# bd4sur/Nano

Measured on AMD Instinct MI355X. Metric: decode_tokens_per_sec, higher is better.
Workload: dtype i8

## Files before the change

### include/nano_mi355x.h

```cpp
#ifndef NANO_MI355X_H
#define NANO_MI355X_H

#include <stddef.h>
#include <stdint.h>

#ifdef __cplusplus
extern "C" {
#endif

#define NANO_ARCH_NANO  0u
#define NANO_ARCH_QWEN2 2u
#define NANO_ARCH_QWEN3 3u

#define NANO_QUANT_F32 0x00u
#define NANO_QUANT_Q80 0x80u
#define NANO_QUANT_Q4K 0x42u

#define NANO_HIP_OK        0
#define NANO_HIP_EINVAL   -1
#define NANO_HIP_ERUNTIME -2
#define NANO_HIP_ENODEV   -3
#define NANO_HIP_ENOMEM   -4

#define NANO_MAX_BATCH 64u
// ... 295 lines not shown
    const float *norm_w;
    const float *attn_part;
    const float *attn_ml;
    uint32_t attn_nsplit, attn_n_head, attn_hd;
    uint32_t use_gemm;
    uint32_t ordered;
    uint32_t *route_out;
    float *out;
    uint32_t out_slots;
    uint32_t out_stride;
    float *tile_max;
    uint32_t tile_slots;
    uint32_t tile_pairs;
    uint32_t *ntiles_out;
    uint32_t *argmax_out;
    const float *resid_add;
    uint32_t resid_add_stride;
} NanoFusedGemvDesc;
int nano_hip_op_fused_gemv(int device, const NanoFusedGemvDesc *d);

typedef struct NanoLoraOpDesc {
    uint32_t E, KD, rank, alpha, nb, S;
    uint32_t v_bstride, _pad;
    const float *x;
    const float *norm_w;
    const float *a[3], *b[3];
    const uint32_t *pos;
    float *q, *kraw, *v;
    uint64_t q_floats, k_floats, v_floats;
} NanoLoraOpDesc;
int nano_hip_op_lora_qkv(int device, const NanoLoraOpDesc *d);
int nano_hip_op_lora_o(int device, const NanoLoraOpDesc *d);
typedef struct NanoLoraAdapter {
    uint32_t rank, alpha;
    const float *a[3], *b[3];
} NanoLoraAdapter;
typedef struct NanoLoraRowsOpDesc {
    uint32_t E, KD, nb, S;
    uint32_t v_bstride, n_adapters;
    const float *x;
    const float *norm_w;
    const NanoLoraAdapter *adapters;
    const uint32_t *row_adapter;
    const uint32_t *pos;
    float *q, *kraw, *v;
    uint64_t q_floats, k_floats, v_floats;
} NanoLoraRowsOpDesc;
int nano_hip_op_lora_qkv_rows(int device, const NanoLoraRowsOpDesc *d);
int nano_hip_op_lora_o_rows(int device, const NanoLoraRowsOpDesc *d);
#define NANO_F32_GEMV_PLAN_WORDS 12
int nano_hip_f32_gemv_plan(const NanoFusedGemvDesc *d, uint32_t cus, uint32_t out[NANO_F32_GEMV_PLAN_WORDS]);
#define NANO_F32_GEMM_PLAN_WORDS 17
int nano_hip_f32_gemm_plan(const NanoFusedGemvDesc *d, uint32_t cus, uint32_t out[NANO_F32_GEMM_PLAN_WORDS]);
#define NANO_Q80_GEMV_PLAN_WORDS 16
int nano_hip_q80_gemv_plan(const NanoFusedGemvDesc *d, uint32_t cus, uint32_t out[NANO_Q80_GEMV_PLAN_WORDS]);
#define NANO_Q80_GEMM_PLAN_WORDS 47
int nano_hip_q80_gemm_plan(const NanoFusedGemvDesc *d, uint32_t cus, uint32_t out[NANO_Q80_GEMM_PLAN_WORDS]);
#define NANO_Q4K_GEMV_PLAN_WORDS 24
int nano_hip_q4k_gemv_plan(const NanoFusedGemvDesc *d, uint32_t cus, uint32_t out[NANO_Q4K_GEMV_PLAN_WORDS]);

#define NANO_QKV_ATTN_FUSED_PLAN_WORDS 16
#define NANO_WO_W13_FUSED_PLAN_WORDS 16
int nano_hip_qkv_attn_fused_plan(const NanoFusedGemvDesc *qkv, const NanoAttnDecodeDesc *attn, uint32_t cus, uint32_t out[NANO_QKV_ATTN_FUSED_PLAN_WORDS]);
int nano_hip_wo_w13_fused_plan(const NanoFusedGemvDesc *wo, const NanoFusedGemvDesc *w13, uint32_t cus, uint32_t out[NANO_WO_W13_FUSED_PLAN_WORDS]);
typedef struct NanoQkvAttnFusedDesc {
    const NanoFusedGemvDesc *qkv;
    const NanoAttnDecodeDesc *attn;
    uint32_t layer1, tick0;
    const unsigned long long *hand_init;
    float *part_out;
    float *ml_out;
    uint32_t *plan_out;
    uint32_t *err_out;
} NanoQkvAttnFusedDesc;
int nano_hip_op_qkv_attn_fused(int device, const NanoQkvAttnFusedDesc *d);
typedef struct NanoWoW13FusedDesc {
    const NanoFusedGemvDesc *wo, *w13;
    uint32_t layer1, tick0;
    const unsigned long long *hand_init;
    uint32_t *plan_out;
    uint32_t *err_out;
} NanoWoW13FusedDesc;
int nano_hip_op_wo_w13_fused(int device, const NanoWoW13FusedDesc *d);

typedef struct NanoBlobShare NanoBlobShare;
int nano_hip_blob_share(NanoBlobShare **out, const void *host_params, size_t bytes, int root_device, const int *devices, int n_devices);
const void *nano_hip_blob_ptr(const NanoBlobShare *s, int i);
void nano_hip_blob_stats(const NanoBlobShare *s, double *upload_s, double *share_s, char *how, size_t how_cap);
void nano_hip_blob_done(NanoBlobShare *s, int i);
void nano_hip_blob_release(NanoBlobShare *s);
int nano_hip_model_device(const NanoHipModel *m);

int nano_hip_stamps_begin(NanoHipModel *m);
int nano_hip_stamps_read(NanoHipModel *m, unsigned long long *out, uint32_t *kinds, uint32_t cap_launches, uint32_t *n_launches);

#ifdef __cplusplus
}
#endif
#endif
```

### nano_amd/binding.py

```python
from __future__ import annotations

import ctypes as C
import os
from typing import Optional, Sequence

import numpy as np

HERE = os.path.dirname(os.path.abspath(__file__))
LIB_PATH = os.environ.get("NANO_LIB") or os.path.join(HERE, "lib", "libnano_mi355x.so")

f32p = np.ctypeslib.ndpointer(dtype=np.float32, flags="C_CONTIGUOUS")
i8p = np.ctypeslib.ndpointer(dtype=np.int8, flags="C_CONTIGUOUS")
u8p = np.ctypeslib.ndpointer(dtype=np.uint8, flags="C_CONTIGUOUS")
u32p = np.ctypeslib.ndpointer(dtype=np.uint32, flags="C_CONTIGUOUS")


class NanoModelDesc(C.Structure):
    _fields_ = [(n, C.c_uint32) for n in (
        "arch", "block_size", "vocab_size", "n_layer", "n_embd", "n_head", "n_kv_head", "n_hidden",
        "is_shared_classifier", "head_dim", "quant_type", "group_size")]


class NanoFusedGemvDesc(C.Structure):
    _fields_ = [("quant", C.c_uint32), ("gs", C.c_uint32), ("kind", C.c_uint32), ("n", C.c_uint32), ("nb", C.c_uint32), ("nseg", C.c_uint32),
# ... 11 lines not shown
                ("q", C.c_void_p), ("kraw", C.c_void_p), ("v", C.c_void_p), ("q_floats", C.c_uint64), ("k_floats", C.c_uint64), ("v_floats", C.c_uint64)]


NANO_LORA_TABLE_MAX = 64
NANO_LORA_NONE = 0xffffffff


class NanoLoraAdapter(C.Structure):
    _fields_ = [("rank", C.c_uint32), ("alpha", C.c_uint32), ("a", C.c_void_p * 3), ("b", C.c_void_p * 3)]


class NanoLoraRowsOpDesc(C.Structure):
    _fields_ = [(n, C.c_uint32) for n in ("E", "KD", "nb", "S", "v_bstride", "n_adapters")] + \
               [("x", C.c_void_p), ("norm_w", C.c_void_p), ("adapters", C.POINTER(NanoLoraAdapter)), ("row_adapter", C.c_void_p), ("pos", C.c_void_p),
                ("q", C.c_void_p), ("kraw", C.c_void_p), ("v", C.c_void_p), ("q_floats", C.c_uint64), ("k_floats", C.c_uint64), ("v_floats", C.c_uint64)]


class NanoAttnDecodeDesc(C.Structure):
    _fields_ = [(n, C.c_uint32) for n in ("nb", "n_head", "n_kv_head", "hd", "n_layer", "layer", "S", "range_hint", "nsplit", "rope_qwen3",
                                          "kv_half", "chunk", "want_frag", "pool_rows", "pt_stride")] + \
               [(n, C.c_void_p) for n in ("q", "k", "vraw", "pos", "q_norm", "k_norm", "rope_cos", "rope_sin", "pt_rows", "k_cache", "v_cache",
                                          "out", "xf", "xsf", "plan")]


class NanoQkvAttnFusedDesc(C.Structure):
    _fields_ = [("qkv", C.POINTER(NanoFusedGemvDesc)), ("attn", C.POINTER(NanoAttnDecodeDesc)), ("layer1", C.c_uint32), ("tick0", C.c_uint32),
                ("hand_init", C.c_void_p), ("part_out", C.c_void_p), ("ml_out", C.c_void_p), ("plan_out", C.c_void_p), ("err_out", C.c_void_p)]


class NanoWoW13FusedDesc(C.Structure):
    _fields_ = [("wo", C.POINTER(NanoFusedGemvDesc)), ("w13", C.POINTER(NanoFusedGemvDesc)), ("layer1", C.c_uint32), ("tick0", C.c_uint32),
                ("hand_init", C.c_void_p), ("plan_out", C.c_void_p), ("err_out", C.c_void_p)]


class NanoExactAttnDesc(C.Structure):
    _fields_ = [(n, C.c_uint32) for n in ("n_head", "n_kv_head", "hd", "S", "range", "is_causal", "long_form", "_pad")] + \
               [(n, C.c_void_p) for n in ("q", "k_cache", "v_cache", "out")]


ATTN_PLAN_FIELDS = ("mode", "lpr", "qv", "kvm", "npt", "w16", "paged", "kv_half", "nsplit", "xcd")


F32_PLAN_FIELDS = ("role", "B", "nv", "upw", "rw", "nw", "grid", "lds_bytes", "launches", "seqs_per_launch", "takes")
F32_PLAN_WORDS = len(F32_PLAN_FIELDS) + 1
F32_ROLES = ("generic", "norm_store", "resid", "resid_combine", "norm_swiglu")


F32_GEMM_PLAN_FIELDS = ("route", "sw", "threads", "grid", "lds_bytes", "rt", "nw", "nt", "nu", "upw", "tp", "stage_bytes", "tab_off",
                        "pro_threads", "pro_lds", "xs_floats", "takes")


Q80_PLAN_FIELDS = ("route", "kernel", "role", "gs", "B", "nv", "upw", "rw", "nw", "grid", "lds_bytes", "variant", "pre", "launches",
                   "seqs_per_launch", "takes")
Q80_ROLES = F32_ROLES
Q80_KERNELS = ("none", "slab", "stream")
Q80_VARIANTS = ("plain", "early", "wf", "wfc2", "wfc3", "wfc4")


Q80_GEMM_PLAN_FIELDS = ("route", "kernel", "tt", "nv", "r", "ms", "tp", "pp", "gs", "sw", "threads", "grid", "lds_bytes", "norm_order",
                        "hh", "ntiles", "tc0", "tc1", "tpw", "full", "nu", "nk", "ttl", "nw", "rounds", "tts", "magic",
                        "nsa", "pre", "a_stage", "a_ws", "b_base", "b_stage", "b_xs", "ks", "ncw", "nss", "tab", "ring", "nl",
                        "waves", "lt", "nhc", "nwaves", "ng", "npass", "takes")
Q80_GEMM_KERNELS = ("none", "g6s", "g6f", "g7", "g7k", "gc", "g2")


Q4K_PLAN_FIELDS = ("route", "kernel", "role", "B", "nv", "ipt", "d", "loop", "rounds", "wg0", "wg1", "wg2", "rw", "nthr", "grid", "lds_bytes",
                   "pre", "quant_rows", "quant_nthr", "quant_nv", "partials", "launches", "seqs_per_launch", "takes")
Q4K_KERNELS = ("none", "slab", "chunk")


QKV_ATTN_FUSED_PLAN_FIELDS = ("kernel", "nv", "upw", "d", "qv", "threads", "n_attn", "ngemv", "lds_bytes", "rw", "wg0", "wg1", "wg2", "rounds",
                              "_zero", "takes")
WO_W13_FUSED_PLAN_FIELDS = ("sig", "threads", "role", "wf", "wfc", "nv_a", "upw_a", "nv_b", "upw_b", "wa", "wb", "lds_bytes", "rw_a", "rw_b",
                            "_zero", "takes")
FUSED_KERNELS = ("none", "q80_table", "q80_wf", "q4k", "f32")
NANO_DEVERR_HANDOFF = 2


ROUTE_NAMES = ("gemv", "gemv_preq", "gemv_sliced", "q4k", "reserved", "frag_g6", "frag_old", "frag_g7", "q4k_gemm", "f32_gemm")


class NanoHipError(RuntimeError):
    pass


class NanoHipTokenScore(C.Structure):
    _fields_ = [("logprob", C.c_float), ("target_logit", C.c_float), ("max_logit", C.c_float), ("lse", C.c_float),
                ("argmax", C.c_uint32), ("rank", C.c_uint32)]


TOKEN_SCORE_DTYPE = np.dtype([("logprob", "<f4"), ("target_logit", "<f4"), ("max_logit", "<f4"), ("lse", "<f4"), ("argmax", "<u4"), ("rank", "<u4")])
assert TOKEN_SCORE_DTYPE.itemsize == C.sizeof(NanoHipTokenScore)


class NanoHipTopEntry(C.Structure):
    _fields_ = [("token", C.c_uint32), ("logit", C.c_float), ("logprob", C.c_float)]


TOP_ENTRY_DTYPE = np.dtype([("token", "<u4"), ("logit", "<f4"), ("logprob", "<f4")])
assert TOP_ENTRY_DTYPE.itemsize == C.sizeof(NanoHipTopEntry) == 12
TOPK_MAX = 32


class NanoHipLookupParams(C.Structure):
    _fields_ = [(n, C.c_uint32) for n in ("max_draft", "ngram_max", "ngram_min", "stop_token", "max_steps")]


class NanoHipPoolParams(C.Structure):
    _fields_ = [(n, C.c_uint32) for n in ("pooling", "normalize", "dim", "reserved")]


POOL_LAST, POOL_MEAN = 0, 1


def _pooling(pooling) -> int:
    return {"last": POOL_LAST, "mean": POOL_MEAN}[pooling] if isinstance(pooling, str) else int(pooling)


class NanoHipLookupStats(C.Structure):
    _fields_ = [(n, C.c_uint32) for n in ("steps_plain", "steps_verify", "drafted", "accepted", "emitted")]


LOOKUP_RECORD_FIELDS = ("emitted", "accepted", "nb_next", "n", "match_len", "match_end", "done", "left")
LOOKUP_NO_STOP = 0xFFFFFFFF


class NanoHipDraftParams(C.Structure):
# ... 687 lines not shown
    check(lib().nano_hip_op_matmul_q80(device, out, np.ascontiguousarray(xq), np.ascontiguousarray(xs),
                                       np.ascontiguousarray(wq), np.ascontiguousarray(ws), n, d, gs)); return out


def op_quantize_q4k(x, device=0):
    x = np.ascontiguousarray(x, np.float32)
    out = np.zeros(((x.size + 255) // 256) * 160, np.uint8)
    check(lib().nano_hip_op_quantize_q4k(device, x, x.size, out)); return out


def op_matmul_q4k(x_blocks, w_blocks, n, d, device=0):
    out = np.empty(d, np.float32)
    check(lib().nano_hip_op_matmul_q4k(device, out, np.ascontiguousarray(x_blocks), np.ascontiguousarray(w_blocks), n, d)); return out


_FLAG = np.zeros(1, np.float32)


def _fused_shape(quant, kind, n, rows, nb, *, gs=0, norm=False, attn=None, ordered=False, use_gemm=False, resid_add=False) -> NanoFusedGemvDesc:
    d = NanoFusedGemvDesc()
    d.quant, d.gs, d.kind, d.n, d.nb, d.nseg = quant, gs, kind, n, nb, len(rows)
    for i, r in enumerate(rows):
        d.rows[i] = r
    if norm:
        d.norm_w = _FLAG.ctypes.data if norm is True else norm
    if attn is not None:
        d.attn_n_head, d.attn_hd, d.attn_nsplit = attn[:3]
        d.attn_part = attn[3] if len(attn) > 3 else _FLAG.ctypes.data
    if resid_add:
        d.resid_add, d.resid_add_stride = (_FLAG.ctypes.data, rows[0]) if resid_add is True else resid_add
    d.ordered = 1 if ordered else 0
    d.use_gemm = 1 if use_gemm else 0
    return d


def _plan_query(name, fields, words, desc, cus):
    assert len(fields) <= words
    out = (C.c_uint32 * words)()
    descs = desc if isinstance(desc, tuple) else (desc,)
    check(getattr(lib(), f"nano_hip_{name}_plan")(*(C.byref(d) for d in descs), cus, out))
    return dict(zip(fields, (int(v) for v in out)))


def f32_gemv_plan(kind, n, rows, nb=1, *, norm=False, attn=None, resid_add=False, cus=256):
    return _plan_query("f32_gemv", F32_PLAN_FIELDS, F32_PLAN_WORDS, _fused_shape(0x00, kind, n, rows, nb, norm=bool(norm), attn=attn, resid_add=bool(resid_add)), cus)


def f32_gemm_plan(kind, n, rows, nb=9, *, norm=False, attn=None, cus=256):
    return _plan_query("f32_gemm", F32_GEMM_PLAN_FIELDS, len(F32_GEMM_PLAN_FIELDS), _fused_shape(0x00, kind, n, rows, nb, norm=bool(norm), attn=attn), cus)


def q80_gemv_plan(kind, n, rows, nb=1, *, gs=64, norm=False, attn=None, ordered=False, use_gemm=False, resid_add=False, cus=256):
    d = _fused_shape(0x80, kind, n, rows, nb, gs=gs, norm=bool(norm), attn=attn, ordered=ordered, use_gemm=use_gemm, resid_add=bool(resid_add))
    return _plan_query("q80_gemv", Q80_PLAN_FIELDS, len(Q80_PLAN_FIELDS), d, cus)


def q80_gemm_plan(kind, n, rows, nb=1, *, gs=64, norm=False, attn=None, ordered=False, use_gemm=False, cus=256):
    d = _fused_shape(0x80, kind, n, rows, nb, gs=gs, norm=bool(norm), attn=attn, ordered=ordered, use_gemm=use_gemm)
    return _plan_query("q80_gemm", Q80_GEMM_PLAN_FIELDS, len(Q80_GEMM_PLAN_FIELDS), d, cus)


def q4k_gemv_plan(kind, n, rows, nb=1, *, norm=False, attn=None, resid_add=False, cus=256):
    return _plan_query("q4k_gemv", Q4K_PLAN_FIELDS, len(Q4K_PLAN_FIELDS), _fused_shape(0x42, kind, n, rows, nb, norm=bool(norm), attn=attn, resid_add=bool(resid_add)), cus)


def op_fused_gemv(quant, kind, n, weights, x=None, norm_w=None, *, gs=0, nb=1, resid=None, attn=None, use_gemm=False, ordered=False,
                  want_route=False, guard=None, partials=None, want_argmax=False, resid_add=None, device=0):
    keep = []

    def held(v, dtype=None):
        v = np.ascontiguousarray(v, dtype); keep.append(v)
        return v

    if norm_w is not None:
        norm_w = held(norm_w, np.float32)
    if attn is not None:
        part, ml, n_head, hd = attn
        part, ml = held(part, np.float32), held(ml, np.float32)
    if resid_add is not None:
        resid_add = held(resid_add, np.float32)
        assert resid_add.ndim == 2 and resid_add.shape[0] == nb
    d = _fused_shape(quant, kind, n, [rows for _, _, rows in weights], nb, gs=gs, norm=norm_w is not None and norm_w.ctypes.data,
                     attn=None if attn is None else (n_head, hd, part.shape[-2], part.ctypes.data), ordered=ordered, use_gemm=use_gemm,
                     resid_add=resid_add is not None and (resid_add.ctypes.data, resid_add.shape[1]))
    for i, (w, ws, _) in enumerate(weights):
        d.w[i] = held(w).ctypes.data
        if ws is not None:
            d.ws[i] = held(ws, np.float32).ctypes.data
    rows_total = weights[0][2] if kind == 2 else sum(r for _, _, r in weights)
    if x is not None:
        d.x = held(x, np.float32).ctypes.data
    if attn is not None:
        d.attn_ml = ml.ctypes.data
    if guard is not None:
        assert resid is None and guard.dtype == np.float32 and guard.flags.c_contiguous and guard.ndim == 2
        out = guard
        d.out_slots, d.out_stride = guard.shape
    else:
        out = np.zeros((nb, rows_total), np.float32) if resid is None else np.array(resid, np.float32, copy=True).reshape(nb, rows_total)
    route = C.c_uint32(0xffffffff)
    d.route_out = C.cast(C.pointer(route), C.c_void_p)
    d.out = out.ctypes.data
    ntiles = C.c_uint32(0xffffffff)
    if partials is not None:
        assert partials.dtype == np.float32 and partials.flags.c_contiguous and partials.ndim == 3 and partials.shape[2] == 2
        d.tile_max, d.tile_slots, d.tile_pairs = partials.ctypes.data, partials.shape[0], partials.shape[1]
        d.ntiles_out = C.cast(C.pointer(ntiles), C.c_void_p)
# ... 561 lines not shown
```

### nano_amd/csrc/backend.hip

```cpp
#include "backend_model.h"

static thread_local std::string g_err;
extern "C" const char *nano_hip_last_error(void) { return g_err.c_str(); }
extern "C" void nano_hip_set_error_(const char *msg) { g_err = msg ? msg : ""; }

extern "C" int nano_hip_device_count(void) {
    int n = 0;
    if (hipGetDeviceCount(&n) != hipSuccess) return 0;
    return n;
}

extern "C" int nano_hip_device_info(int device, char *name, size_t cap, uint64_t *total_mem) {
    hipDeviceProp_t p;
    HIP_TRY(hipGetDeviceProperties(&p, device));
    if (name && cap) { strncpy(name, p.gcnArchName, cap - 1); name[cap - 1] = 0; }
    if (total_mem) *total_mem = p.totalGlobalMem;
    return p.multiProcessorCount;
}

struct Piece { size_t src_off, bytes, dst_off; };

static void shapes(const NanoModelDesc &d, uint32_t &hd, uint32_t &QD, uint32_t &KD) {
    if (d.arch == NANO_ARCH_QWEN3) { hd = d.head_dim; QD = hd * d.n_head; KD = hd * d.n_kv_head; }
    else { hd = d.n_embd / d.n_head; QD = d.n_embd; KD = (d.n_embd * d.n_kv_head) / d.n_head; }
// ... 229 lines not shown
    m->nsplit_cap = max_seq_len > attention_wide_from() ? attention_split_cap() : 8;
    bool ok = hipMalloc(&m->x, Bs * E * 4) == hipSuccess && hipMalloc(&m->q, Bs * QD * 4) == hipSuccess &&
              hipMalloc(&m->kraw, Bs * KD * 4) == hipSuccess && hipMalloc(&m->xba, Bs * QD * 4) == hipSuccess &&
              hipMalloc(&m->hb, Bs * H * 4) == hipSuccess && hipMalloc(&m->logits, B * V * 4) == hipSuccess &&
              hipMalloc(&m->kcache, kvn * kv_esz(m)) == hipSuccess && hipMalloc(&m->vcache, kvn * kv_esz(m)) == hipSuccess &&
              (!m->kv_half || hipMalloc(&m->vraw, Bs * KD * 4) == hipSuccess) &&
              hipMalloc(&m->tokens, Bs * 4) == hipSuccess && hipMalloc(&m->pos, Bs * 4) == hipSuccess &&
              hipMalloc(&m->amax, B * 4) == hipSuccess && hipMalloc(&m->trace, (size_t)m->trace_cap * 4) == hipSuccess &&
              hipMalloc(&m->pos0, B * 4) == hipSuccess &&
              hipMalloc(&m->attn_part, Bs * m->nsplit_cap * QD * 4) == hipSuccess &&
              hipMalloc(&m->attn_ml, Bs * d.n_head * m->nsplit_cap * 2 * 4) == hipSuccess &&
              hipMalloc(&m->tile_max, B * V * 2 * 4) == hipSuccess &&
              hipMalloc(&m->rope_cur, Bs * m->hd * 4 + 64) == hipSuccess;
    if (ok && Bs > 8 && d.quant_type == NANO_QUANT_Q80) {
        size_t nmax = E > QD ? E : QD; if (H > nmax) nmax = H;
        ok = hipMalloc(&m->gq, Bs * ((nmax + 15) & ~(size_t)15)) == hipSuccess && hipMalloc(&m->gxs, Bs * (nmax / d.group_size) * 4) == hipSuccess;
    }
    if (ok && Bs > 1 && d.quant_type == NANO_QUANT_Q4K) {
        size_t nmax = E > QD ? E : QD; if (H > nmax) nmax = H;
        m->q4x_bytes = (Bs > 8 ? (Bs < 64 ? Bs : (size_t)64) : (size_t)8) * ((nmax + 255) & ~(size_t)255);
        ok = hipMalloc(&m->q4x, m->q4x_bytes) == hipSuccess;
    }
    if (ok && Bs > 8 && f32 && m->f32_min_nb <= 64u) {
        size_t nmax = E > QD ? E : QD; if (H > nmax) nmax = H;
        m->f32x_floats = (size_t)64 * ((nmax + 127) & ~(size_t)127);
        ok = hipMalloc(&m->f32x, m->f32x_floats * 4) == hipSuccess;
    }
    if (ok && m->kv.paged) {
        const size_t ptn = B * m->kv.pt_stride;
        ok = hipMalloc(&m->kv.pt, ptn * 4) == hipSuccess && hipMalloc(&m->kv.kvrow, Bs * 4) == hipSuccess && hipHostMalloc(&m->kv.h_pt, ptn * 4) == hipSuccess &&
             hipMemset(m->kv.pt, 0xff, ptn * 4) == hipSuccess && hipMemset(m->kv.kvrow, 0, Bs * 4) == hipSuccess;
        if (ok) {
            memset(m->kv.h_pt, 0xff, ptn * 4);
            for (uint32_t pg = m->kv.pages; pg-- > 0;) m->kv.free_pages.push_back(pg);
            m->kv.page_owners.assign(m->kv.pages, 0u);
        }
    }
    if (!ok) { destroy(m); FAIL(NANO_HIP_ENOMEM, "hipMalloc for KV cache / scratch failed (batch %zu, seq %u)", B, max_seq_len); }
    if (hipMemset(m->kcache, 0, kvn * kv_esz(m)) != hipSuccess || hipMemset(m->vcache, 0, kvn * kv_esz(m)) != hipSuccess ||
        hipMemset(m->x, 0, Bs * E * 4) != hipSuccess || hipMemset(m->logits, 0, B * V * 4) != hipSuccess ||
        hipMemset(m->tokens, 0, Bs * 4) != hipSuccess || hipMemset(m->pos, 0, Bs * 4) != hipSuccess ||
        hipMemset(m->pos0, 0, B * 4) != hipSuccess) { destroy(m); FAIL(NANO_HIP_ERUNTIME, "hipMemset failed"); }
    ok = hipHostMalloc(&m->h_tokens, Bs * 4) == hipSuccess && hipHostMalloc(&m->h_pos, Bs * 4) == hipSuccess &&
         hipHostMalloc(&m->h_amax, (size_t)m->trace_cap * 4) == hipSuccess && hipHostMalloc(&m->h_logits, B * V * 4) == hipSuccess;
    if (!ok) { destroy(m); FAIL(NANO_HIP_ENOMEM, "hipHostMalloc failed"); }
    if (hipHostMalloc(reinterpret_cast<void **>(&m->h_err), 64, hipHostMallocMapped) != hipSuccess ||
        hipHostGetDevicePointer(reinterpret_cast<void **>(&m->dev_err), m->h_err, 0) != hipSuccess) { destroy(m); FAIL(NANO_HIP_ENOMEM, "hipHostMalloc (mapped) failed"); }
    *m->h_err = 0;
    if (hipStreamCreateWithFlags(&m->st, hipStreamNonBlocking) != hipSuccess || hipEventCreate(&m->ev0) != hipSuccess ||
        hipEventCreate(&m->ev1) != hipSuccess || hipEventCreate(&m->ev2) != hipSuccess) { destroy(m); FAIL(NANO_HIP_ERUNTIME, "stream/event creation failed"); }
    if (getenv("NANO_HIP_NO_GRAPH")) m->use_graph = false;
    if (const char *nt = getenv("NANO_KV_COPY_NT")) m->kv.copy_nt = *nt && *nt != '0';
    if (const char *fz = getenv("NANO_FUSE_LAUNCHES")) { const uint32_t v = (uint32_t)strtoul(fz, nullptr, 0); m->ho.fuse_qkv_attn = (v & 1u) != 0; m->ho.fuse_wo_w13 = (v & 2u) != 0; }
    {
        const bool gran = (m->d.quant_type == NANO_QUANT_Q80 && m->d.group_size == 64) || m->d.quant_type == NANO_QUANT_Q4K || m->d.quant_type == NANO_QUANT_F32;
        const size_t g1 = gran ? (size_t)m->QD + 2 * (size_t)m->KD : 0, g2 = (gran && m->d.quant_type == NANO_QUANT_Q80) ? (size_t)m->d.n_embd : 0;
        if (handoff_alloc(&m->ho.tick, &m->ho.hand, g1, &m->ho.hand2, g2) != hipSuccess) { destroy(m); FAIL(NANO_HIP_ENOMEM, "hipMalloc of the hand-off words and granules failed"); }
    }
    HIP_TRY(hipDeviceSynchronize());
    *out = m;
    if (const char *xm = getenv("NANO_EXACT")) if (*xm && *xm != '0') { const int rc = nano_hip_set_exact(m, 1); if (rc) return rc; }
    if (const char *sm = getenv("NANO_STRICT")) if (*sm && *sm != '0') return nano_hip_set_strict(m, 1);
    return NANO_HIP_OK;
}

extern "C" int nano_hip_model_device(const NanoHipModel *m) { return m ? m->device : -1; }
extern "C" uint64_t nano_hip_weight_bytes_per_step(const NanoHipModel *m) { return m ? m->weight_bytes_per_step : 0; }
hipError_t nano::handoff_alloc(uint32_t **tick, unsigned long long **hand, size_t granules, unsigned long long **hand2, size_t granules2) {
    hipError_t e;
    if ((e = hipMalloc(reinterpret_cast<void **>(tick), 64)) != hipSuccess || (e = hipMemset(*tick, 0, 64)) != hipSuccess) return e;
    if (granules && ((e = hipMalloc(reinterpret_cast<void **>(hand), granules * 8)) != hipSuccess || (e = hipMemset(*hand, 0, granules * 8)) != hipSuccess)) return e;
    if (granules2 && ((e = hipMalloc(reinterpret_cast<void **>(hand2), granules2 * 8)) != hipSuccess || (e = hipMemset(*hand2, 0, granules2 * 8)) != hipSuccess)) return e;
    return hipSuccess;
}
uint32_t dev_err_take(NanoHipModel *m) {
    const uint32_t c = m->h_err ? *reinterpret_cast<volatile uint32_t *>(m->h_err) : 0u;
    if (!c) return 0u;
    *reinterpret_cast<volatile uint32_t *>(m->h_err) = 0;
    m->ho.last_dev_err = c;
    if (m->ho.tick) (void)hipMemsetAsync(m->ho.tick + 2, 0, 4, m->st);
    return c;
}
int dev_err_fail(uint32_t c) {
    FAIL(NANO_HIP_ERUNTIME, "a kernel gave up waiting for its producers (code %u: 1 = G6 tile counter, 2 = in-launch hand-off of a fused launch): the results of this call are not valid", c);
}
int dev_err_check(NanoHipModel *m) {
    const uint32_t c = dev_err_take(m);
    return c ? dev_err_fail(c) : 0;
}
void drop_graphs(NanoHipModel *m) {
    for (auto &kv : m->graphs) (void)hipGraphExecDestroy(kv.second);
    m->graphs.clear(); m->pf_graph_keys.clear(); m->exact_nodes.clear();
}
void handoff_fallback(NanoHipModel *m) {
    (void)hipStreamSynchronize(m->st);
    m->ho.fuse_qkv_attn = m->ho.fuse_wo_w13 = false;
    drop_graphs(m);
    m->ho.fallbacks++;
}

extern "C" int nano_hip_sync(NanoHipModel *m) {
    if (!m) FAIL(NANO_HIP_EINVAL, "null model");
    HIP_TRY(hipSetDevice(m->device));
    HIP_TRY(hipStreamSynchronize(m->st));
    return dev_err_check(m);
}
// ... 290 lines not shown
```

### nano_amd/csrc/backend_model.h

```cpp
#pragma once
#include <math.h>
#include <stdio.h>
#include <stdlib.h>
#include <string.h>

#include <map>
#include <string>
#include <utility>
#include <vector>

#include <hip/hip_fp16.h>
#include "../../include/nano_mi355x.h"
#include "kernels.h"
#include "kv_image.h"
#include "pool_plan.h"
#include "step_spec.h"

using namespace nano;
extern "C" void nano_hip_set_error_(const char *msg);

#define HIP_TRY(expr)                                                                              \
    do {                                                                                           \
        hipError_t _e = (expr);                                                                    \
        if (_e != hipSuccess) {                                                                    \
// ... 53 lines not shown
    uint32_t f32_min_nb = 9;
    uint32_t pf_chunk = 8;
    float *rope_cur = nullptr;
    float *kcache = nullptr, *vcache = nullptr;
    uint32_t *tokens = nullptr, *pos = nullptr, *amax = nullptr, *trace = nullptr, *pos0 = nullptr;
    uint32_t trace_cap = 0, nsplit = 1;
    uint32_t nsplit_cap = 8;
    uint32_t *h_tokens = nullptr, *h_pos = nullptr, *h_amax = nullptr;
    struct RowScratch {
        float *logits = nullptr;
        ScorePartial *part = nullptr;
        uint32_t *targets = nullptr;
        NanoHipTokenScore *rows = nullptr;
        uint32_t *amax = nullptr;
        unsigned long long *keys = nullptr;
        uint8_t *call = nullptr; uint32_t cap = 0, have = 0;
        uint32_t *tok = nullptr, *pos = nullptr, *slot = nullptr;
        uint32_t *tgt = nullptr, *out_amax = nullptr;
        NanoHipTokenScore *sc = nullptr;
        NanoHipTopEntry *top = nullptr;
        uint32_t *pool_map = nullptr;
        float *pool_acc = nullptr, *pool_out = nullptr;
    } rb;
    struct Lookup {
        uint32_t *hist = nullptr; uint32_t cap = 0;
        std::vector<uint32_t> shadow;
        uint32_t *state = nullptr;
        uint32_t *h_rec = nullptr;
        bool graph = true;
    } lk;
    struct Draft {
        uint32_t *iota = nullptr;
        hipEvent_t ev_t = nullptr, ev_d = nullptr;
        bool timing = false;
        hipEvent_t tm[4] = {nullptr, nullptr, nullptr, nullptr};
        double ms[3] = {0, 0, 0}; uint32_t timed = 0;
    } dr;
    struct Rows {
        using Group = RowGroup;
        float *vraw = nullptr;
    } rows;
    uint32_t *h_err = nullptr, *dev_err = nullptr;
    float *h_logits = nullptr;
    std::map<uint64_t, hipGraphExec_t> graphs;
    std::vector<uint64_t> pf_graph_keys;
    uint64_t weight_bytes_per_step = 0;
    bool use_graph = true;
    uint32_t mfma_min_nb = 9;
    struct Handoff {
        bool fuse_qkv_attn = true;
        unsigned long long *hand = nullptr;
        bool fuse_wo_w13 = true;
        unsigned long long *hand2 = nullptr;
        uint32_t *tick = nullptr;
        uint32_t fallbacks = 0;
        bool reissue = true;
        uint32_t last_dev_err = 0;
    } ho;
    std::vector<uint32_t> fw_tokens, fw_pos; uint32_t fw_causal = 0; int fw_logits = 0, fw_argmax = 0;
    Sampler *smp = nullptr;
    uint32_t rope_rows = 0;
    uint32_t pending_batch = 0;
    uint32_t kv_half = 0;
    float *vraw = nullptr;
    struct PagedKv {
        bool paged = false;
        uint32_t pages = 0, pt_stride = 0;
        uint32_t *pt = nullptr, *kvrow = nullptr;
        uint32_t *h_pt = nullptr;
        std::vector<uint32_t> free_pages;
        std::vector<uint32_t> page_owners;
        uint64_t cow_copies = 0;
        std::vector<std::vector<uint32_t>> pt_stage;
        uint32_t *jobs = nullptr; size_t jobs_cap = 0;
        bool copy_nt = false;
    } kv;
    bool strict = false;
    float *xn = nullptr, *hb2 = nullptr, *att = nullptr;
    nano_hip_phase_fn phase_fn = nullptr; void *phase_env = nullptr;
    bool exact = false;
    std::map<uint64_t, uint32_t> exact_nodes;
    uint32_t exact_launches = 0;
    struct Stamps {
        unsigned long long *buf = nullptr; uint32_t launches = 0; bool on = false;
        std::vector<uint32_t> kinds;
    } stamp;
    struct KvImageIo {
        uint8_t *dev = nullptr, *host = nullptr;
        size_t half = 0; uint32_t chunk_blocks = 0;
        hipStream_t cp = nullptr;
        hipEvent_t staged[2] = {nullptr, nullptr};
        hipEvent_t freed[2] = {nullptr, nullptr};
        uint32_t *jobs = nullptr; size_t jobs_cap = 0;
    } kvi;
    uint64_t params_bytes = 0;
};

inline size_t align_up(size_t v, size_t a) { return (v + a - 1) / a * a; }
inline size_t kv_esz(const NanoHipModel *m) { return kv_fmt_bytes(m->kv_half); }
inline uint64_t weight_bytes(uint32_t quant, uint32_t gs, uint64_t n_weights) {
    return quant == NANO_QUANT_F32 ? 4 * n_weights : quant == NANO_QUANT_Q80 ? n_weights + 4 * (n_weights / gs) : n_weights * 160 / 256;
}

uint32_t dev_err_take(NanoHipModel *m);
int dev_err_fail(uint32_t c);
int dev_err_check(NanoHipModel *m);
// ... 109 lines not shown
```

### nano_amd/csrc/backend_step.hip

```cpp
#include "backend_model.h"

namespace nano { extern hipEvent_t g_q80_probe_start, g_q80_probe_stop; }

static unsigned long long *next_stamps(NanoHipModel *m, uint32_t kind) {
    if (!m->stamp.on || m->stamp.launches >= STAMP_MAX_LAUNCHES) return nullptr;
    m->stamp.kinds.push_back(kind);
    return m->stamp.buf + (size_t)(m->stamp.launches++) * STAMP_WGS * 8;
}

static GemvSeg mkseg(const TensorRef &t, float *out, uint32_t rows, uint32_t bstride, uint32_t pstride = 0) {
    GemvSeg s{}; s.w = t.w; s.ws = t.s; s.out = out; s.rows = rows; s.out_bstride = bstride; s.out_pstride = pstride;
    return s;
}
static Q80Route route_of(const NanoHipModel *m) {
    Q80Route r{};
    r.quant = m->d.quant_type; r.cus = m->cus; r.mfma_min_nb = m->mfma_min_nb;
    r.gq = m->gq; r.gxs = m->gxs; r.q4x = m->q4x; r.q4x_bytes = m->q4x_bytes;
    r.f32_min_nb = m->f32_min_nb; r.f32x = m->f32x; r.f32x_floats = m->f32x_floats;
    return r;
}
static RouteKind kind_of(const NanoHipModel *m, GemvArgs a) { a.ordered = (m->strict || m->exact) ? 1u : 0u; a.cus = (uint32_t)m->cus; return route_kind(route_of(m), a); }

static hipError_t gemv(NanoHipModel *m, GemvArgs &a) {
    a.ordered = (m->strict || m->exact) ? 1u : 0u;
    a.err = m->dev_err;
    return route_projection(route_of(m), a, m->st);
}

static GemvArgs classifier_args(const NanoHipModel *m, uint32_t nb, float *dst) {
    GemvArgs a{};
    a.nseg = 1; a.seg[0] = mkseg(m->cls, dst, m->d.vocab_size, m->d.vocab_size);
    a.n = m->d.n_embd; a.gs = m->d.group_size; a.nb = nb; a.xin = m->x; a.xin_bstride = m->d.n_embd;
    a.epi = GEMV_EPI_STORE; a.norm_w = m->rms_final; a.pos = m->pos;
    return a;
}

hipError_t enqueue_classifier(NanoHipModel *m, uint32_t nb, uint32_t *ntiles_out, float *dst) {
    GemvArgs a = classifier_args(m, nb, dst ? dst : m->logits);
    a.ordered = (m->strict || m->exact) ? 1u : 0u;
    if (ntiles_out)
        if (const uint32_t n = route_partials(route_of(m), a)) { a.tile_max = m->tile_max; *ntiles_out = n; }
    return gemv(m, a);
}
hipError_t enqueue_score_rows(NanoHipModel *m, const float *logits, uint32_t rows, const uint32_t *targets, NanoHipTokenScore *out) {
    ScoreArgs a{};
    a.logits = logits; a.V = m->d.vocab_size; a.ntiles = score_tiles(a.V); a.targets = targets; a.part = m->rb.part; a.out = out;
    return launch_score_rows(a, rows, m->st);
}
static uint32_t step_nsplit(const NanoHipModel *m, uint32_t nb, uint32_t range_hint) {
    uint32_t ns = attention_nsplit(range_hint, m->hd);
    if (nb >= 4) { const uint32_t div = nb / 2; ns = (ns + div - 1) / div; }
    if (nb >= m->mfma_min_nb) ns = 1;
    if (m->lora_on) ns = 1;
    if (nb > 1 && (uint64_t)(m->d.n_embd / 16) * nb * m->QD > (4u << 20)) ns = 1;
    return ns ? ns : 1;
}

static GemvArgs proj_args(const NanoHipModel *m, uint32_t nb, uint32_t n, const float *xin, uint32_t epi) {
    GemvArgs a{};
    a.n = n; a.gs = m->d.group_size; a.nb = nb; a.xin = xin; a.xin_bstride = n; a.epi = epi; a.pos = m->pos;
    return a;
}
static GemvArgs qkv_args(const NanoHipModel *m, uint32_t l, uint32_t nb, const float *xin, const float *norm_w, const KvRows::VTarget &v) {
    GemvArgs a = proj_args(m, nb, m->d.n_embd, xin, GEMV_EPI_STORE);
    a.nseg = 3;
    a.seg[0] = mkseg(m->W[WQ][l], m->q, m->QD, m->QD);
    a.seg[1] = mkseg(m->W[WK][l], m->kraw, m->KD, m->KD);
    a.seg[2] = mkseg(m->W[WV][l], v.out, m->KD, v.bstride, v.pstride);
    a.norm_w = norm_w; a.pos = v.pos;
    return a;
}
static GemvArgs wo_args(const NanoHipModel *m, uint32_t l, uint32_t nb, uint32_t nsplit) {
    GemvArgs a = proj_args(m, nb, m->QD, m->xba, GEMV_EPI_RESID);
    a.nseg = 1; a.seg[0] = mkseg(m->W[WO][l], m->x, m->d.n_embd, m->d.n_embd);
    if (m->lora_on) { a.resid_add = m->lora_o1; a.resid_add_bstride = m->d.n_embd; }
    if (nsplit > 1) { a.attn_part = m->attn_part; a.attn_ml = m->attn_ml; a.attn_nsplit = nsplit; a.attn_n_head = m->d.n_head; a.attn_hd = m->hd; }
    return a;
}
static GemvArgs w13_args(const NanoHipModel *m, uint32_t l, uint32_t nb, const float *xin, const float *norm_w, float *w3_out, uint32_t epi) {
    GemvArgs a = proj_args(m, nb, m->d.n_embd, xin, epi);
    a.nseg = 2; a.seg[0] = mkseg(m->W[W1][l], m->hb, m->d.n_hidden, m->d.n_hidden); a.seg[1] = mkseg(m->W[W3][l], w3_out, m->d.n_hidden, m->d.n_hidden);
    a.norm_w = norm_w;
    return a;
}
static LoraRowsArgs lora_rows_args(const NanoHipModel *m, const StepSpec &s, uint32_t l) {
    LoraRowsArgs a{};
    a.desc = m->lt.desc; a.E = m->d.n_embd; a.KD = m->KD; a.layer = l; a.slot0 = s.slot; a.slot_stride = s.one_slot() ? 0u : 1u; a.max_rank = m->lt.max_rank;
    return a;
}
static GemvArgs w2_args(const NanoHipModel *m, uint32_t l, uint32_t nb) {
    GemvArgs a = proj_args(m, nb, m->d.n_hidden, m->hb, GEMV_EPI_RESID);
    a.nseg = 1; a.seg[0] = mkseg(m->W[W2][l], m->x, m->d.n_embd, m->d.n_embd);
    return a;
}
static bool wo_takes_parts(const NanoHipModel *m, const StepSpec &s, uint32_t nsplit) {
    const uint32_t nb = s.nb;
    if (nsplit <= 1 || nsplit > 8 || s.rows_split_alone()) return false;
    if (route_takes_fragments(kind_of(m, wo_args(m, 0, nb, 1)))) return false;
    return route_takes_attn_parts(kind_of(m, wo_args(m, 0, nb, nsplit)));
}
static uint32_t spec_nsplit(const NanoHipModel *m, const StepSpec &s) { return step_nsplit(m, s.rows_split_alone() ? 1u : s.nb, s.range_hint); }
uint32_t xba_nsplit(const NanoHipModel *m, const StepSpec &s, bool ordered) {
    if (s.rows != StepSpec::SEQS || ordered) return 1u;
    const uint32_t ns = spec_nsplit(m, s);
    return (ns > 1 && !wo_takes_parts(m, s, ns)) ? 1u : ns;
}
static const uint32_t *paged_rows(const NanoHipModel *m, const StepSpec &s) { return m->kv.pt + (s.one_slot() ? (size_t)s.slot * m->kv.pt_stride : 0); }
static uint32_t paged_bstride(const NanoHipModel *m, const StepSpec &s) { return s.rows_split_alone() ? 0u : m->kv.pt_stride; }
static EmbedArgs embed_args(const NanoHipModel *m, const StepSpec &s) {
    EmbedArgs ea{};
    ea.tok = m->tok.w; ea.tok_s = m->tok.s; ea.tokens = m->tokens; ea.x = m->x;
    ea.E = m->d.n_embd; ea.gs = m->d.group_size; ea.quant = m->d.quant_type; ea.x_bstride = m->d.n_embd;
    ea.rope_cos = m->rope_cos; ea.rope_sin = m->rope_sin; ea.pos = m->pos; ea.rope_cur = m->rope_cos ? m->rope_cur : nullptr; ea.half = m->hd / 2;
    if (m->kv.paged) { ea.pt_rows = paged_rows(m, s); ea.kvrow = m->kv.kvrow; ea.pt_bstride = paged_bstride(m, s); ea.pt_entries = m->kv.pt_stride; }
    ea.row_slot = s.row_slot;
    return ea;
}
static ArgmaxArgs argmax_args(const NanoHipModel *m, uint32_t nb, const float *logits, uint32_t *amax) {
    ArgmaxArgs aa{};
    aa.logits = logits; aa.V = m->d.vocab_size; aa.bstride = m->d.vocab_size; aa.out = amax; aa.pos = m->pos; aa.pos0 = m->pos0; aa.nb = nb;
    return aa;
}
static AttnArgs attn_args(const NanoHipModel *m, const StepSpec &s, const KvRows &kv, uint32_t l, uint32_t nsplit) {
    const NanoModelDesc &d = m->d;
    AttnArgs a{};
    a.err = m->dev_err;
    a.q = m->q; a.kraw = m->kraw; kv.attention(a); a.pos = m->pos;
    a.q_norm = m->q_norm ? m->q_norm + (size_t)l * m->hd : nullptr;
    a.k_norm = m->k_norm ? m->k_norm + (size_t)l * m->hd : nullptr;
// ... 323 lines not shown
```

### nano_amd/csrc/gemv_common.h

```cpp
#pragma once
#define NANO_GEMV_COMMON_H 1
#include <stdlib.h>
#include "device_common.h"
#include "kernels.h"

namespace nano {

namespace {

#define DPP_I(v, ctrl) __builtin_amdgcn_update_dpp(0, (v), (ctrl), 0xF, 0xF, true)
#define DPP_F(v, ctrl) __int_as_float(__builtin_amdgcn_update_dpp(0, __float_as_int(v), (ctrl), 0xF, 0xF, true))

template <int W> __device__ __forceinline__ int dpp_group_sum(int v) {
    if (W >= 2) v += DPP_I(v, 0xB1);
    if (W >= 4) v += DPP_I(v, 0x4E);
    if (W >= 8) v += DPP_I(v, 0x141);
    if (W >= 16) v += DPP_I(v, 0x140);
    return v;
}
template <int W> __device__ __forceinline__ float dpp_group_max(float v) {
    if (W >= 2) v = fmaxf(v, DPP_F(v, 0xB1));
    if (W >= 4) v = fmaxf(v, DPP_F(v, 0x4E));
    if (W >= 8) v = fmaxf(v, DPP_F(v, 0x141));
    if (W >= 16) v = fmaxf(v, DPP_F(v, 0x140));
// ... 38 lines not shown
    const int8_t *w[3]; const float *ws[3]; float *out[3];
    uint32_t rows[3], out_bstride[3], out_pstride[3];
    uint32_t n, ng, rw, log2_tiles, nchunk, magic_nchunk, units, epi, flags, nb;
    uint32_t tpw, magic_rw, wg_c0, wg_c1;
    const float *xin; const float *norm_w; const uint32_t *pos;
    uint32_t xin_bstride, nthr;
    const int8_t *xq_in; const float *xs_in;
    const float *attn_part; const float *attn_ml;
    uint32_t attn_nsplit, attn_n_head, attn_hd, ntiles;
    float *tile_max;
    const float *resid_add; uint32_t resid_add_bstride;
    uint32_t early;
    unsigned long long *stamps;
    uint32_t dbg;
    uint32_t canon;
    uint32_t *err;
};

struct QkvAttnArgs { GemvDev g; AttnArgs a; SlabHand hand; uint32_t n_attn, head_wgs, wait16, ngemv; };
static inline uint32_t fused_attn_wgs(const AttnArgs &aa) { return aa.n_head * aa.nsplit; }
static inline size_t fused_attn_lds(uint32_t hd, bool plain) {
    const size_t hd4 = (hd + 3) & ~3u;
    return (hd4 + hd4 + 4 + 4 + 4 * hd4 + hd4 + (plain ? 0 : 4 + 4 * 8 * hd4)) * sizeof(float);
}
static void fused_attn_setup(QkvAttnArgs &fa, const AttnArgs &aa, unsigned long long *hand, uint32_t *tick, uint32_t layer1) {
    AttnArgs &a = fa.a;
    a = aa;
    { uint32_t l2 = 0; while ((1u << l2) < a.n_kv_head) l2++; a.kv_log2 = l2; }
    { const uint32_t kv_mul = a.n_head / a.n_kv_head; uint32_t l2 = 0; while ((1u << l2) < kv_mul) l2++; a.kvmul_log2 = l2; }
    fa.hand.buf = hand; fa.hand.tick = tick; fa.hand.layer1 = layer1;
    fa.hand.base[0] = 0; fa.hand.base[1] = a.q_dim; fa.hand.base[2] = a.q_dim + a.kv_dim;
    fa.n_attn = fused_attn_wgs(a); fa.head_wgs = a.n_head;
}

template <int ROLE> __device__ __forceinline__ bool has_flag(const GemvDev &a, uint32_t f) {
    if (ROLE == R_GENERIC) return (a.flags & f) != 0;
    if (f == F_NORM) return ROLE == R_NORM_STORE || ROLE == R_NORM_SWIGLU;
    if (f == F_COMBINE) return ROLE == R_RESID_COMBINE;
    return false;
}
template <int ROLE> __device__ __forceinline__ uint32_t role_epi(const GemvDev &a) {
    if (ROLE == R_GENERIC) return a.epi;
    if (ROLE == R_NORM_STORE) return GEMV_EPI_STORE;
    if (ROLE == R_NORM_SWIGLU) return GEMV_EPI_SWIGLU;
    return GEMV_EPI_RESID;
}

template <int B, int NV>
struct Staged {
    float4 x[B][NV];
    float4 nw[NV];
    float4 pv[B == 1 ? NV : 1][B == 1 ? 8 : 1];
    float ml_m, ml_l;
};
template <int B>
struct Staged<B, 0> {};

template <int ROLE, int B, int NV>
__device__ __forceinline__ void stage_issue(const GemvDev &a, Staged<B, NV> &r) {
    if constexpr (NV == 0) { (void)a; (void)r; return; } else {
    const uint32_t tid = threadIdx.x, nthr = a.nthr, n = a.n;
    const bool plain = !has_flag<ROLE>(a, F_PRE) && !has_flag<ROLE>(a, F_COMBINE);
    const __amdgpu_buffer_rsrc_t rx = mkrsrc(a.xin, plain ? ((a.nb - 1) * a.xin_bstride + n) * 4u : 0u);
    const __amdgpu_buffer_rsrc_t rn = mkrsrc(a.norm_w, has_flag<ROLE>(a, F_NORM) ? n * 4u : 0u);
#pragma unroll
    for (int j = 0; j < NV; j++) {
        const uint32_t i = (tid + (uint32_t)j * nthr) * 4u;
        const uint32_t off = (i < n) ? i * 4u : OOB;
        if (plain) {
#pragma unroll
            for (int b = 0; b < B; b++) r.x[b][j] = bload_f4(rx, (b < (int)a.nb) ? off + (uint32_t)b * a.xin_bstride * 4u : OOB);
        }
        if (has_flag<ROLE>(a, F_NORM)) r.nw[j] = (NANO_STAMPS && (a.dbg & 1u)) ? make_float4(1.f, 1.f, 1.f, 1.f) : bload_f4(rn, off);
    }
    if constexpr (B == 1) {
      if (has_flag<ROLE>(a, F_COMBINE)) {
        const uint32_t ns = a.attn_nsplit, nh = a.attn_n_head;
        const __amdgpu_buffer_rsrc_t rp = mkrsrc(a.attn_part, ns * n * 4u);
        const __amdgpu_buffer_rsrc_t rm = mkrsrc(a.attn_ml, nh * ns * 8u);
#pragma unroll
        for (int j = 0; j < NV; j++) {
            const uint32_t i = (tid + (uint32_t)j * nthr) * 4u;
#pragma unroll
            for (int sp = 0; sp < 8; sp++) r.pv[j][sp] = bload_f4(rp, (i < n && (uint32_t)sp < ns) ? ((uint32_t)sp * n + i) * 4u : OOB);
        }
        const uint32_t sp = tid & 7u, h = tid >> 3;
        const uint32_t mo = (h < nh && sp < ns) ? (h * ns + sp) * 8u : OOB;
        r.ml_m = bload_f(rm, mo);
        r.ml_l = bload_f(rm, mo == OOB ? OOB : mo + 4u);
      }
    }
    }
}

template <int ROLE, int B, int NV>
__device__ __forceinline__ void stage_issue_nw(const GemvDev &a, Staged<B, NV> &r) {
    if constexpr (NV == 0) { (void)a; (void)r; return; } else {
    const uint32_t tid = threadIdx.x, nthr = a.nthr, n = a.n;
    const __amdgpu_buffer_rsrc_t rn = mkrsrc(a.norm_w, has_flag<ROLE>(a, F_NORM) ? n * 4u : 0u);
#pragma unroll
    for (int j = 0; j < NV; j++) {
        const uint32_t i = (tid + (uint32_t)j * nthr) * 4u;
        if (has_flag<ROLE>(a, F_NORM)) r.nw[j] = bload_f4(rn, (i < n) ? i * 4u : OOB);
    }
    }
}

template <int B, bool PRE>
__device__ __forceinline__ void combine_weights(const GemvDev &a, float *wgt , float pm, float pl) {
    const uint32_t tid = threadIdx.x, nthr = a.nthr;
    const uint32_t ns = a.attn_nsplit, nh = a.attn_n_head;
    for (uint32_t t = tid; t < (uint32_t)B * nh * 8u; t += nthr) {
        const uint32_t s = t & 7u, h = (t >> 3) % nh, b = (t >> 3) / nh;
// ... 74 lines not shown
```

### nano_amd/csrc/gemv_q80.hip

```cpp
#include "gemv_q80_host.h"

namespace nano {

hipEvent_t g_q80_probe_start = nullptr, g_q80_probe_stop = nullptr;

hipError_t launch_gemv_q80_gs32(const GemvArgs &a, const Q80GemvPlan &p, hipStream_t st);
hipError_t launch_gemv_q80_gs64(const GemvArgs &a, const Q80GemvPlan &p, hipStream_t st);
hipError_t launch_gemv_q80_gs128(const GemvArgs &a, const Q80GemvPlan &p, hipStream_t st);
hipError_t launch_gemv_q80_gs256(const GemvArgs &a, const Q80GemvPlan &p, hipStream_t st);

uint32_t gemv_q80_partials(const GemvArgs &a) { return use_stream(a) ? STREAM_WGS * 4 : 0; }

SlabPlan q80_plan_slab(const GemvArgs &a, int B) {
    const uint32_t nchunk = (a.n + 1023) / 1024, nmat = a.epi == GEMV_EPI_SWIGLU ? 2 : 1;
    const uint32_t nseg = a.epi == GEMV_EPI_SWIGLU ? 1u : a.nseg;
    uint32_t align = 0;
    if (nseg > 1) for (uint32_t s = 0; s < nseg; s++) align |= a.seg[s].rows;
    const uint32_t rows = gemv_total_rows(a);
    uint32_t rw = 4;
    while (rw < 32 && (align % (rw * 2)) == 0 && (rw * 2 / 4) * nchunk <= 4 && rows / (rw * 2) >= 128) rw *= 2;
    while (rw < 64 && (align % (rw * 2)) == 0 && rows / (rw * 2) >= 256) rw *= 2;
    {
        const uint32_t ng = a.n / a.gs, pitch = ((ng + 47) / 64) * 64 + 16;
        while (rw > 4 && (size_t)B * nmat * rw * pitch * 4 > 64 * 1024) rw /= 2;
// ... 58 lines not shown
        p.kernel = Q80_KERNEL_STREAM;
        p.role = f == F_NORM ? (uint32_t)R_NORM_STORE : (uint32_t)R_GENERIC;
        const uint32_t nvr = (a.n + 1023) / 1024;
        p.nv = nvr <= 1 ? 1u : (B <= 4 && nvr <= 2) ? 2u : (B <= 2 && nvr <= 4) ? 4u : 0u;
        p.upw = 0; p.rw = 16; p.nw = 4; p.grid = STREAM_WGS;
        const uint64_t lds = act + 4ull * 16 * (1024 / a.gs) * 4;
        if (lds > GEMV_Q80_LDS_MAX) return false;
        p.lds_bytes = (uint32_t)lds;
        if (out) *out = p;
        return true;
    }
    const SlabPlan sp = q80_plan_slab(a, (int)B);
    if (sp.upw > 4) return false;
    p.kernel = Q80_KERNEL_SLAB;
    p.rw = sp.rw; p.nw = sp.nw;
    p.nv = sp.nv <= 1 ? 1u : sp.nv <= 2 ? 2u : sp.nv <= 4 ? 4u : 0u;
    if (B * p.nv > 8) p.nv = 0;
    p.upw = sp.upw <= 1 ? 1u : sp.upw <= 2 ? 2u : 4u;
    const bool sw = a.epi == GEMV_EPI_SWIGLU;
    const uint32_t nmat = sw ? 2u : 1u, nseg = sw ? 1u : a.nseg;
    p.early = (B <= 2 && sp.upw >= 2 && (uint64_t)rows * a.n * nmat >= (8u << 20)) ? 1u : 0u;
    const uint32_t tpw = (sp.rw + 3) / 4, nchunk = (a.n + 1023) / 1024;
    p.units = tpw * nchunk * nmat;
    uint32_t wg[3] = {0, 0, 0};
    for (uint32_t s = 0; s < nseg; s++) wg[s] = (a.seg[s].rows + sp.rw - 1) / sp.rw;
    p.wg_c0 = nseg > 1 ? wg[0] : 0xffffffffu;
    p.wg_c1 = nseg > 2 ? wg[0] + wg[1] : 0xffffffffu;
    p.grid = wg[0] + wg[1] + wg[2];
    p.role = R_GENERIC;
    if (B == 1 && (a.gs != 64 || q80_canonical(a))) {
        if (f == F_NORM && a.epi == GEMV_EPI_STORE) p.role = R_NORM_STORE;
        else if (f == 0 && a.epi == GEMV_EPI_RESID) p.role = R_RESID;
        else if (f == F_COMBINE && a.epi == GEMV_EPI_RESID) p.role = R_RESID_COMBINE;
        else if (f == F_NORM && a.epi == GEMV_EPI_SWIGLU) p.role = R_NORM_SWIGLU;
    }
    const uint64_t pitch = (1024 / a.gs == 16) ? (((ng + 47) / 64) * 64 + 16) : (ng4 + 4);
    const uint64_t comb = (f & F_COMBINE) ? (uint64_t)B * a.attn_n_head * 32 : 0;
    uint64_t lds = act + comb + (uint64_t)B * nmat * (tpw * 4) * pitch * 4;
    GemvDev d = to_dev(a);
    d.early = p.early; d.tpw = tpw;
    p.variant = Q80_VAR_PLAIN;
    if (a.gs == 64 && B <= 2 && p.upw >= 2 && p.nv >= 1 && p.early) p.variant = Q80_VAR_EARLY;
    else if (a.gs == 64 && B == 1 && (p.role == R_NORM_STORE || p.role == R_NORM_SWIGLU) && (p.nv == 1 || p.nv == 2) && slab_wave_fold(d)) {
        p.variant = Q80_VAR_WF;
        if (p.role == R_NORM_SWIGLU) p.units = (sp.rw + 1) / 2;
        lds = n16 + ng4 * 4 + 64;
    } else if (a.gs == 64 && B == 1 && (p.role == R_RESID || p.role == R_RESID_COMBINE) && (p.nv == 1 || p.nv == 2) && p.upw <= 2) {
        const uint32_t nch = slab_wave_fold_chunks(d);
        if (nch) {
            p.variant = nch == 2u ? Q80_VAR_WFC2 : nch == 3u ? Q80_VAR_WFC3 : Q80_VAR_WFC4;
            lds = n16 + ng4 * 4 + 64 + comb + slab_unit_table(d, nch);
        }
    }
    if (lds > GEMV_Q80_LDS_MAX) return false;
    p.lds_bytes = (uint32_t)lds;
    if (out) *out = p;
    return true;
}

uint32_t gemv_q80_fit_batch(const GemvArgs &a) {
    GemvArgs t = a;
    for (uint32_t c = 8; c >= 1; c >>= 1) { t.nb = c; if (gemv_q80_plan(t, nullptr)) return c; }
    return 0;
}

hipError_t launch_gemv_q80(const GemvArgs &a, hipStream_t st) {
    Q80GemvPlan p;
    if (!gemv_q80_plan(a, &p)) return hipErrorInvalidValue;
    switch (a.gs) {
    case 32: return launch_gemv_q80_gs32(a, p, st);
    case 64: return launch_gemv_q80_gs64(a, p, st);
    case 128: return launch_gemv_q80_gs128(a, p, st);
    case 256: return launch_gemv_q80_gs256(a, p, st);
    default: return hipErrorInvalidValue;
    }
}

}
```

### nano_amd/csrc/gemv_q80_host.h

```cpp
#pragma once
#include "kernels.h"
#include "gemv_common.h"
#include <hip/hip_ext.h>
#include <stdlib.h>

namespace nano {

constexpr uint32_t STREAM_MIN_ROWS = 16384;
static inline uint32_t stream_wgs() { return 1024u; }
#define STREAM_WGS (::nano::stream_wgs())

static inline bool use_stream(const GemvArgs &a) {
    return a.nseg == 1 && a.epi == GEMV_EPI_STORE && a.seg[0].rows >= STREAM_MIN_ROWS && a.seg[0].out_pstride == 0 && !a.attn_part && a.nb <= 8;
}

struct SlabPlan { uint32_t rw, nw, upw, nv; };
SlabPlan q80_plan_slab(const GemvArgs &a, int B);

static inline bool slab_wave_fold(const GemvDev &d) {
    return d.n == 1024u && d.ng == 16u && !d.early && (d.epi == GEMV_EPI_STORE || (d.epi == GEMV_EPI_SWIGLU && !d.out_pstride[0]));
}
static inline uint32_t slab_wave_fold_chunks(const GemvDev &d) {
    if (d.nb != 1u || d.early || d.epi != GEMV_EPI_RESID || d.resid_add || d.out_pstride[0] || d.rows[1] || (d.flags & ~F_COMBINE)) return 0u;
    if (d.n % 1024u || d.n < 2048u || d.n > 4096u || d.ng * 64u != d.n) return 0u;
    return d.n / 1024u;
}
static inline size_t slab_unit_table(const GemvDev &d, uint32_t nch) { return (size_t)(d.tpw * 4) * (nch <= 2u ? 4u : 8u) * 4u; }

extern hipEvent_t g_q80_probe_start, g_q80_probe_stop;

}
```

### nano_amd/csrc/gemv_q80_impl.h

```cpp
#include <string.h>
#include <stdio.h>
#include "gemv_common.h"
#include "gemv_q80_host.h"

namespace nano {

namespace {


__device__ __forceinline__ void quant_store4(float4 v, float scale, int8_t *dst) {
    *reinterpret_cast<uint32_t *>(dst) = q80_pack4(q80_quant4(v, scale));
}

template <int ROLE, int GS, int B, int NV>
__device__ __forceinline__ void stage_finish(const GemvDev &a, Staged<B, NV> &r, int8_t *xq, float *xs, float *red, uint32_t n16, uint32_t ng4) {
    const uint32_t tid = threadIdx.x, nthr = a.nthr, n = a.n, ng = a.ng;
    const uint32_t lane = tid & 63u, wid = tid >> 6, NW = nthr >> 6;
    if (has_flag<ROLE>(a, F_PRE)) {
        for (uint32_t b = 0; b < a.nb; b++) {
            for (uint32_t i = tid * 16u; i < n; i += nthr * 16u) *reinterpret_cast<int4 *>(xq + b * n16 + i) = *reinterpret_cast<const int4 *>(a.xq_in + (size_t)b * n16 + i);
            for (uint32_t i = tid; i < ng; i += nthr) xs[b * ng4 + i] = a.xs_in[(size_t)b * ng + i];
        }
        __syncthreads();
        return;
    }
    const bool norm = has_flag<ROLE>(a, F_NORM), comb = has_flag<ROLE>(a, F_COMBINE);
    float *wgt = red + B * 16;
    if constexpr (NV == 0) {
        if (comb) combine_weights<B, false>(a, wgt, 0.0f, 0.0f);
        for (uint32_t b = 0; b < a.nb; b++) {
            const float *x = a.xin + (size_t)b * a.xin_bstride;
            float ss = 1.0f;
            if (norm) {
                float acc = 0.0f;
                for (uint32_t i = tid * 4u; i < n; i += nthr * 4u) {
                    const float4 v = comb ? combine4(a, b, i, wgt) : *reinterpret_cast<const float4 *>(x + i);
                    acc += v.x * v.x; acc += v.y * v.y; acc += v.z * v.z; acc += v.w * v.w;
                }
                acc = dpp_wave_sum(acc);
                __syncthreads();
                if (lane == 0) red[wid] = acc;
                __syncthreads();
                float t = 0.0f;
                for (uint32_t w = 0; w < NW; w++) t += red[w];
                t /= (float)n; t += 1e-5f;
                ss = 1.0f / sqrtf(t);
            }
            for (uint32_t i = tid * 4u; i < n; i += nthr * 4u) {
                float4 v = comb ? combine4(a, b, i, wgt) : *reinterpret_cast<const float4 *>(x + i);
                if (norm) {
                    const float4 w = *reinterpret_cast<const float4 *>(a.norm_w + i);
                    v.x = w.x * (ss * v.x); v.y = w.y * (ss * v.y); v.z = w.z * (ss * v.z); v.w = w.w * (ss * v.w);
                }
                float m = fmaxf(fmaxf(fabsf(v.x), fabsf(v.y)), fmaxf(fabsf(v.z), fabsf(v.w)));
                m = dpp_group_max<GS / 4>(m);
                const float scale = div_const<127>(m);
                quant_store4(v, scale, xq + b * n16 + i);
                if ((tid % (GS / 4)) == 0) xs[b * ng4 + i / GS] = scale;
            }
        }
        __syncthreads();
    } else {
        if (comb) {
            if constexpr (B == 1) {
                const bool pre_ml = a.attn_n_head * 8u <= nthr;
                if (pre_ml) combine_weights<B, true>(a, wgt, r.ml_m, r.ml_l); else combine_weights<B, false>(a, wgt, 0.0f, 0.0f);
#pragma unroll
                for (int j = 0; j < NV; j++) {
                    const uint32_t i = (tid + (uint32_t)j * nthr) * 4u;
                    const float *wg = wgt + (size_t)((i < n ? i : 0u) / a.attn_hd) * 8u;
                    float4 acc = make_float4(0.f, 0.f, 0.f, 0.f);
#pragma unroll
                    for (int sp = 0; sp < 8; sp++) {
                        const float w = wg[sp];
                        acc.x += r.pv[j][sp].x * w; acc.y += r.pv[j][sp].y * w; acc.z += r.pv[j][sp].z * w; acc.w += r.pv[j][sp].w * w;
                    }
                    r.x[0][j] = acc;
                }
            } else {
                combine_weights<B, false>(a, wgt, 0.0f, 0.0f);
#pragma unroll
                for (int b = 0; b < B; b++)
#pragma unroll
                    for (int j = 0; j < NV; j++) {
                        const uint32_t i = (tid + (uint32_t)j * nthr) * 4u;
                        r.x[b][j] = (i < n && b < (int)a.nb) ? combine4(a, b, i, wgt) : make_float4(0.f, 0.f, 0.f, 0.f);
                    }
            }
        }
        float ss[B];
#pragma unroll
        for (int b = 0; b < B; b++) ss[b] = 1.0f;
        if (norm) {
#pragma unroll
            for (int b = 0; b < B; b++) {
                float acc = 0.0f;
#pragma unroll
                for (int j = 0; j < NV; j++) {
                    acc += r.x[b][j].x * r.x[b][j].x; acc += r.x[b][j].y * r.x[b][j].y;
                    acc += r.x[b][j].z * r.x[b][j].z; acc += r.x[b][j].w * r.x[b][j].w;
                }
                acc = dpp_wave_sum(acc);
                if (lane == 0) red[b * 16 + wid] = acc;
            }
            __syncthreads();
#pragma unroll
            for (int b = 0; b < B; b++) {
                float t = 0.0f;
                for (uint32_t w = 0; w < NW; w++) t += red[b * 16 + w];
                t /= (float)n; t += 1e-5f;
                ss[b] = 1.0f / sqrtf(t);
            }
        }
        NANO_STAMP(a.stamps, 2, ss[0] + r.x[0][0].x);
#pragma unroll
// ... 136 lines not shown

template <int ROLE, int GS, int B, int NV, int UPW, int EARLY = 0, int WF = 0, int WFC = 0>
__global__ __launch_bounds__(1024) void gemv_q80_slab_kernel(const GemvDev a) {
    extern __shared__ __attribute__((aligned(16))) unsigned char smem[];
#define SLAB_EARLY EARLY
#define SLAB_WF WF
#define SLAB_WFC WFC
#define SLAB_A a
#define SLAB_BID blockIdx.x
#define SLAB_HAND 0
#define SLAB_HANDV (SlabHand{})
#define SLAB_PTAG 0u
#define SLAB_XHAND 0
#define SLAB_XHANDV (SlabHand{})
#define SLAB_CTAG 0u
#define SLAB_PART 0
#include "gemv_q80_slab_body.inc"
#undef SLAB_A
#undef SLAB_BID
#undef SLAB_HAND
#undef SLAB_HANDV
#undef SLAB_PTAG
#undef SLAB_XHAND
#undef SLAB_XHANDV
#undef SLAB_CTAG
#undef SLAB_PART
#undef SLAB_EARLY
#undef SLAB_WF
#undef SLAB_WFC
}

#if NANO_Q80_GS == 64
}
}
#include "attn_impl.h"
namespace nano {
namespace {
template <int NV, int UPW>
__global__ __launch_bounds__(256) void qkv_attn_fused_kernel(const QkvAttnArgs fa) {
#define SLAB_WF 0
#include "qkv_attn_fused_body.inc"
#undef SLAB_WF
}
__global__ __launch_bounds__(256) void qkv_attn_fused_wf_kernel(const QkvAttnArgs fa) {
    constexpr int NV = 1, UPW = 1;
#define SLAB_WF 1
#include "qkv_attn_fused_body.inc"
#undef SLAB_WF
}

struct Wo13Args { GemvDev wo; GemvDev w13; SlabHand hand; uint32_t wo_wgs, wait16; };
template <int ROLE_A, int WF, int WFA>
__global__ __launch_bounds__(512) void wo_w13_fused_kernel(const Wo13Args fa) {
    extern __shared__ __attribute__((aligned(16))) unsigned char smem[];
    constexpr int GS = 64, B = 1, NV = 1, UPW = 1;
    const uint2 tk_ = hand_tick(fa.hand);
    {
        constexpr int ROLE = ROLE_A;
#define SLAB_BID blockIdx.x
#define SLAB_A fa.wo
#define SLAB_HAND 1
#define SLAB_HANDV fa.hand
#define SLAB_PTAG hand_ptag(tk_, fa.hand)
#define SLAB_XHAND 0
#define SLAB_XHANDV (SlabHand{})
#define SLAB_CTAG 0u
#define SLAB_WFC WFA
#define SLAB_PART 1
#include "gemv_q80_slab_body.inc"
#undef SLAB_PART
        auto wo_rest = [&]() __attribute__((always_inline)) {
#define SLAB_PART 2
#include "gemv_q80_slab_body.inc"
#undef SLAB_PART
        };
#undef SLAB_WFC
#undef SLAB_A
#undef SLAB_HAND
#undef SLAB_HANDV
#undef SLAB_PTAG
#undef SLAB_XHAND
#undef SLAB_XHANDV
#undef SLAB_CTAG
        {
            constexpr int ROLE = R_NORM_SWIGLU;
#define SLAB_A fa.w13
#define SLAB_HAND 0
#define SLAB_HANDV (SlabHand{})
#define SLAB_PTAG 0u
#define SLAB_XHAND 1
#define SLAB_XHANDV fa.hand
#define SLAB_CTAG hand_ctag(tk_, fa.hand)
#define SLAB_XHAND_WAIT (blockIdx.x >= fa.wo_wgs ? fa.wait16 : 0u)
#define SLAB_XHAND_NAP 2
#define SLAB_WF WF
#define SLAB_PART 1
#include "gemv_q80_slab_body.inc"
#undef SLAB_PART
            if (blockIdx.x < fa.wo_wgs) wo_rest();
            __syncthreads();
#define SLAB_PART 2
#include "gemv_q80_slab_body.inc"
#undef SLAB_PART
#undef SLAB_A
#undef SLAB_HAND
#undef SLAB_HANDV
#undef SLAB_PTAG
#undef SLAB_XHAND
#undef SLAB_XHANDV
#undef SLAB_CTAG
#undef SLAB_XHAND_WAIT
#undef SLAB_XHAND_NAP
#undef SLAB_WF
        }
#undef SLAB_BID
    }
}

#endif

template <int ROLE, int GS, int B, int NV>
__global__ __launch_bounds__(256) void gemv_q80_stream_kernel(const GemvDev a) {
    extern __shared__ __attribute__((aligned(16))) unsigned char smem[];
    constexpr int LPG = GS / 16, GC = 1024 / GS, F = GC / 4;
    static_assert(F >= 1, "group size too large for the stream kernel");
    const uint32_t n = a.n, ng = a.ng;
    const int tid = threadIdx.x, lane = tid & 63;
    const int wid = __builtin_amdgcn_readfirstlane(tid >> 6);
    const uint32_t n16 = (n + 15) & ~15u, ng4 = (ng + 3) & ~3u;
    int8_t *xq = reinterpret_cast<int8_t *>(smem);
    float *xs = reinterpret_cast<float *>(smem + B * n16);
    float *red = xs + B * ng4;
    int *tab = reinterpret_cast<int *>(red + B * 16) + wid * 16 * GC;

    Staged<B, NV> sx;
    stage_issue<ROLE, B, NV>(a, sx);

    const uint32_t rows = a.rows[0];
    const uint32_t nchunk = a.nchunk;
    const uint32_t ntiles = (rows + 15) >> 4;
    const uint32_t nwaves = gridDim.x * 4, wave_g = blockIdx.x * 4 + (uint32_t)wid;
    const uint32_t nunits = (wave_g < ntiles) ? ((ntiles - wave_g + nwaves - 1) / nwaves) * nchunk : 0;
    const __amdgpu_buffer_rsrc_t rw_ = mkrsrc(a.w[0], rows * n);
    const __amdgpu_buffer_rsrc_t rs_ = mkrsrc(a.ws[0], rows * ng * 4u);

    int4 wA[16];
    float sA[F];
    uint32_t tile_i = 0, chunk_i = 0;
    auto issue = [&](int4 (&w)[16], float (&s)[F]) {
        const uint32_t tile = wave_g + tile_i * nwaves;
        const uint32_t row0 = tile << 4;
        const uint32_t col = (chunk_i << 10) + (uint32_t)lane * 16u;
        const uint32_t base = (col < n) ? row0 * n + col : OOB;
#pragma unroll
        for (int r = 0; r < 16; r++) w[r] = bload_w(rw_, base + (uint32_t)r * n);
        const uint32_t gb = chunk_i * GC + ((uint32_t)lane & 3u) * F;
        const uint32_t so = ((row0 + ((uint32_t)lane >> 2)) * ng + gb) * 4u;
#pragma unroll
        for (int f = 0; f < F; f++) s[f] = bload_f(rs_, (gb + f < ng) ? so + 4u * f : OOB);
        if (++chunk_i == nchunk) { chunk_i = 0; tile_i++; }
    };
    if (nunits) issue(wA, sA);

    stage_finish<ROLE, GS, B, NV>(a, sx, xq, xs, red, n16, ng4);

    float val[B], best[B];
    uint32_t besti[B];
#pragma unroll
    for (int b = 0; b < B; b++) { val[b] = 0.0f; best[b] = -INFINITY; besti[b] = 0xffffffffu; }
// ... 37 lines not shown
                    cur = (st == 0) ? DPP_F(t, 0x00) : (st == 1) ? DPP_F(t, 0x55) : (st == 2) ? DPP_F(t, 0xAA) : DPP_F(t, 0xFF);
                }
                val[b] = cur;
                if (last) {
                    if ((lane & 3) == 0 && row < rows) {
                        a.out[0][(size_t)b * a.out_bstride[0] + row] = cur;
                        if (cur > best[b] || besti[b] == 0xffffffffu) { best[b] = cur; besti[b] = row; }
                    }
                    val[b] = 0.0f;
                }
            }
        }
        if (++cchunk == nchunk) { cchunk = 0; ctile++; }
    };
    for (uint32_t u = 0; u < nunits; u++) {
        if (u) issue(wA, sA);
        consume(wA, sA);
    }
    if (a.tile_max) {
#pragma unroll
        for (int b = 0; b < B; b++) {
            if (b < (int)a.nb) {
                float bv = best[b]; uint32_t bi = besti[b];
#pragma unroll
                for (int o = 32; o >= 4; o >>= 1) {
                    const float ov = __shfl_xor(bv, o, 64);
                    const uint32_t oi = __shfl_xor(bi, o, 64);
                    if (oi != 0xffffffffu && (bi == 0xffffffffu || ov > bv || (ov == bv && oi < bi))) { bv = ov; bi = oi; }
                }
                if (lane == 0) {
                    float *tm = a.tile_max + ((size_t)b * a.ntiles + wave_g) * 2;
                    tm[0] = bv; tm[1] = __uint_as_float(bi);
                }
            }
        }
    }
}


template <int ROLE, int GS, int B, int NV, int UPW>
static hipError_t launch_slab_t(const GemvDev &d, const Q80GemvPlan &p, hipStream_t st) {
    GemvDev dd = d; dd.nthr = 64 * p.nw;
    const size_t lds = p.lds_bytes;
    if constexpr (GS == 64 && B <= 2 && UPW >= 2 && NV >= 1) if (p.variant == Q80_VAR_EARLY) {
        auto kern = &gemv_q80_slab_kernel<ROLE, GS, B, NV, UPW, 1>;
        if (lds > 64 * 1024) (void)hipFuncSetAttribute(reinterpret_cast<const void *>(kern), hipFuncAttributeMaxDynamicSharedMemorySize, (int)lds);
        hipLaunchKernelGGL(kern, dim3(p.grid), dim3(64 * p.nw), lds, st, dd);
        return hipGetLastError();
    }
    if constexpr (GS == 64 && B == 1 && (ROLE == R_NORM_STORE || ROLE == R_NORM_SWIGLU) && (NV == 1 || NV == 2)) if (p.variant == Q80_VAR_WF) {
        hipLaunchKernelGGL((gemv_q80_slab_kernel<ROLE, GS, B, NV, UPW, 0, 1>), dim3(p.grid), dim3(64 * p.nw), lds, st, dd);
        return hipGetLastError();
    }
    if constexpr (GS == 64 && B == 1 && (ROLE == R_RESID || ROLE == R_RESID_COMBINE) && (NV == 1 || NV == 2) && UPW <= 2) {
        if (p.variant == Q80_VAR_WFC2) { hipLaunchKernelGGL((gemv_q80_slab_kernel<ROLE, GS, B, NV, UPW, 0, 0, 2>), dim3(p.grid), dim3(64 * p.nw), lds, st, dd); return hipGetLastError(); }
        if (p.variant == Q80_VAR_WFC3) { hipLaunchKernelGGL((gemv_q80_slab_kernel<ROLE, GS, B, NV, UPW, 0, 0, 3>), dim3(p.grid), dim3(64 * p.nw), lds, st, dd); return hipGetLastError(); }
        if (p.variant == Q80_VAR_WFC4) { hipLaunchKernelGGL((gemv_q80_slab_kernel<ROLE, GS, B, NV, UPW, 0, 0, 4>), dim3(p.grid), dim3(64 * p.nw), lds, st, dd); return hipGetLastError(); }
    }
    if (p.variant != Q80_VAR_PLAIN) return hipErrorInvalidValue;
    auto kern = &gemv_q80_slab_kernel<ROLE, GS, B, NV, UPW>;
    if (lds > 64 * 1024) (void)hipFuncSetAttribute(reinterpret_cast<const void *>(kern), hipFuncAttributeMaxDynamicSharedMemorySize, (int)lds);
    hipLaunchKernelGGL(kern, dim3(p.grid), dim3(64 * p.nw), lds, st, dd);
    return hipGetLastError();
}
template <int ROLE, int GS, int B>
static hipError_t launch_slab_r(const GemvDev &d, const Q80GemvPlan &p, hipStream_t st) {
#define SLAB_GO(NV_, UPW_) do { if constexpr (B * NV_ <= 8) { if (p.nv == NV_ && p.upw == UPW_) return launch_slab_t<ROLE, GS, B, NV_, UPW_>(d, p, st); } } while (0)
    SLAB_GO(1, 1); SLAB_GO(1, 2); SLAB_GO(1, 4);
    SLAB_GO(2, 1); SLAB_GO(2, 2); SLAB_GO(2, 4);
    SLAB_GO(4, 1); SLAB_GO(4, 2); SLAB_GO(4, 4);
    SLAB_GO(0, 1); SLAB_GO(0, 2); SLAB_GO(0, 4);
    return hipErrorInvalidValue;
#undef SLAB_GO
}
template <int GS, int B>
static hipError_t launch_slab_b(GemvDev &d, const Q80GemvPlan &p, hipStream_t st) {
    d.rw = p.rw;
    d.early = p.early;
    d.tpw = (p.rw + 3) / 4;
    d.magic_rw = 65536u / p.rw + 1u;
    d.log2_tiles = 0;
    d.units = p.units;
    d.wg_c0 = p.wg_c0; d.wg_c1 = p.wg_c1;
    if constexpr (B == 1) {
        if (p.role == R_NORM_STORE) return launch_slab_r<R_NORM_STORE, GS, B>(d, p, st);
        if (p.role == R_RESID) return launch_slab_r<R_RESID, GS, B>(d, p, st);
        if (p.role == R_RESID_COMBINE) return launch_slab_r<R_RESID_COMBINE, GS, B>(d, p, st);
        if (p.role == R_NORM_SWIGLU) return launch_slab_r<R_NORM_SWIGLU, GS, B>(d, p, st);
    }
    if (p.role != R_GENERIC) return hipErrorInvalidValue;
    return launch_slab_r<R_GENERIC, GS, B>(d, p, st);
}

template <int ROLE, int GS, int B>
static hipError_t launch_stream_r(GemvDev &d, const Q80GemvPlan &p, hipStream_t st) {
    d.ntiles = p.grid * 4; d.nthr = 64 * p.nw;
    const size_t lds = p.lds_bytes;
    hipEvent_t e0 = g_q80_probe_start, e1 = g_q80_probe_stop;
    g_q80_probe_start = g_q80_probe_stop = nullptr;
#define STREAM_GO(NV_) do { auto kern = &gemv_q80_stream_kernel<ROLE, GS, B, NV_>; \
                            if (lds > 64 * 1024) (void)hipFuncSetAttribute(reinterpret_cast<const void *>(kern), hipFuncAttributeMaxDynamicSharedMemorySize, (int)lds); \
                            if (e0 && e1) hipExtLaunchKernelGGL(kern, dim3(p.grid), dim3(64 * p.nw), (uint32_t)lds, st, e0, e1, 0, d); \
                            else hipLaunchKernelGGL(kern, dim3(p.grid), dim3(64 * p.nw), lds, st, d); return hipGetLastError(); } while (0)
    if (p.nv == 1) STREAM_GO(1);
    if constexpr (B <= 4) { if (p.nv == 2) STREAM_GO(2); }
    if constexpr (B <= 2) { if (p.nv == 4) STREAM_GO(4); }
// ... 8 lines not shown
    return launch_stream_r<R_GENERIC, GS, B>(d, p, st);
}

#if NANO_Q80_GS == 64
static bool fused_shape(const GemvArgs &ga, const AttnArgs &aa, QkvAttnFusedPlan &f) {
    if (ga.gs != 64 || ga.nb != 1 || ga.nseg != 3 || ga.epi != GEMV_EPI_STORE || !ga.norm_w || ga.xq_in || ga.attn_part || ga.tile_max || ga.resid_add) return false;
    if (ga.n % 64u || ga.n > 4096u || use_stream(ga) || !q80_canonical(ga)) return false;
    if (ga.seg[0].out_pstride || ga.seg[1].out_pstride) return false;
    const SlabPlan p = q80_plan_slab(ga, 1);
    if (p.nw != 4u || p.upw > 4u) return false;
    const GemvDev d = to_dev(ga);
    const bool wf = slab_wave_fold(d);
    const uint32_t upw = p.upw <= 1 ? 1u : p.upw <= 2 ? 2u : 4u;
    if (wf ? p.nv != 1u || upw != 1u : !(p.nv == 1u || (p.nv == 2u && upw <= 2u))) return false;
    if (!fused_attn_side_ok(aa, ga.seg[0].rows, ga.seg[1].rows, ga.seg[2].rows, false)) return false;
    f = QkvAttnFusedPlan{};
    f.kernel = wf ? FUSED_KERNEL_Q80_WF : FUSED_KERNEL_Q80_TABLE;
    f.nv = p.nv; f.upw = upw;
    f.threads = 256; f.rw = p.rw;
    for (uint32_t s2 = 0; s2 < 3; s2++) { f.wg[s2] = (ga.seg[s2].rows + p.rw - 1) / p.rw; f.ngemv += f.wg[s2]; }
    f.n_attn = fused_attn_wgs(aa);
    const uint32_t tpw = (p.rw + 3) / 4;
    const size_t n16 = (d.n + 15) & ~15u, ng4 = (d.ng + 3) & ~3u, pitch = ((d.ng + 47) / 64) * 64 + 16;
    const size_t lds_g = n16 + ng4 * 4 + 64 + (wf ? 0 : (size_t)(tpw * 4) * pitch * 4), lds_a = fused_attn_lds(aa.hd, false);
    const size_t lds = lds_g > lds_a ? lds_g : lds_a;
    if (lds > FUSED_LDS_MAX) return false;
    f.lds_bytes = (uint32_t)lds;
    return true;
}

struct Wo13Plan { SlabPlan a, b; uint32_t wa, wb; };
static bool wo13_slabs(const GemvArgs &wo, const GemvArgs &w13, Wo13Plan &q) {
    if (wo.gs != 64 || w13.gs != 64 || wo.nb != 1 || w13.nb != 1 || !q80_canonical(wo) || !q80_canonical(w13)) return false;
    if (wo.nseg != 1 || wo.epi != GEMV_EPI_RESID || wo.norm_w || wo.xq_in || wo.tile_max || wo.resid_add || wo.seg[0].out_pstride) return false;
    if (wo.attn_part && (wo.attn_nsplit > 8u || wo.attn_hd % 4u)) return false;
    if (w13.nseg != 2 || w13.epi != GEMV_EPI_SWIGLU || !w13.norm_w || w13.xq_in || w13.attn_part || w13.tile_max || w13.resid_add) return false;
    if (use_stream(wo) || use_stream(w13) || w13.n != wo.seg[0].rows || w13.xin != wo.seg[0].out || w13.n % 4u) return false;
    q.a = q80_plan_slab(wo, 1); q.b = q80_plan_slab(w13, 1);
    q.wa = (wo.seg[0].rows + q.a.rw - 1) / q.a.rw; q.wb = (w13.seg[0].rows + q.b.rw - 1) / q.b.rw;
    const uint32_t cus = w13.cus ? w13.cus : 256u;
    if (q.wa > q.wb || q.wb > cus) return false;
    const uint32_t units_a = ((q.a.rw + 3) / 4) * ((wo.n + 1023) / 1024), items_a = wo.n / 4;
    const uint32_t units_b = ((q.b.rw + 3) / 4) * ((w13.n + 1023) / 1024) * 2u, items_b = w13.n / 4;
    return q.b.nw == 4u && q.b.nv == 1u && q.b.upw == 2u && units_b <= 8u && items_b >= 1u && items_b <= 512u &&
           items_a > 256u && items_a <= 512u && units_a >= 1u && units_a <= 4u;
}
static void slab_dev_fill(GemvDev &d, const GemvArgs &a, const SlabPlan &p, uint32_t nthr) {
    d.tile_max = nullptr;
    d.rw = p.rw; d.tpw = (p.rw + 3) / 4; d.magic_rw = 65536u / p.rw + 1u; d.log2_tiles = 0;
    d.units = d.tpw * d.nchunk * (a.epi == GEMV_EPI_SWIGLU ? 2u : 1u);
    d.wg_c0 = 0xffffffffu; d.wg_c1 = 0xffffffffu;
    d.nthr = nthr;
}
static size_t slab_lds(const GemvDev &d, bool table = true) {
    const uint32_t nmat = d.epi == GEMV_EPI_SWIGLU ? 2 : 1;
    const size_t n16 = (d.n + 15) & ~15u, ng4 = (d.ng + 3) & ~3u, pitch = ((d.ng + 47) / 64) * 64 + 16;
    return n16 + ng4 * 4 + 64 + ((d.flags & F_COMBINE) ? (size_t)d.attn_n_head * 32 : 0) + (table ? (size_t)nmat * (d.tpw * 4) * pitch * 4 : 0);
}
static bool wo13_shape(const GemvArgs &wo, const GemvArgs &w13, WoW13FusedPlan &f, GemvDev &da, GemvDev &db) {
    Wo13Plan q;
    if (!wo13_slabs(wo, w13, q)) return false;
    da = to_dev(wo); db = to_dev(w13);
    slab_dev_fill(da, wo, q.a, 512); slab_dev_fill(db, w13, q.b, 512);
    const bool wf = slab_wave_fold(db);
    if (wf) db.units = (db.rw + 1) / 2;
    const bool wfa = slab_wave_fold_chunks(da) == 2u;
    const size_t la = slab_lds(da, !wfa) + (wfa ? slab_unit_table(da, 2u) : 0), lb = slab_lds(db, !wf), lds = la > lb ? la : lb;
    if (lds > FUSED_LDS_MAX) return false;
    f = WoW13FusedPlan{};
    f.sig = 3; f.threads = 512;
    f.role = (da.flags & F_COMBINE) ? (uint32_t)R_RESID_COMBINE : (uint32_t)R_RESID;
    f.wf = wf ? 1u : 0u; f.wfc = wfa ? 2u : 0u;
    f.nv_a = 1; f.upw_a = 1; f.nv_b = 1; f.upw_b = 1;
    f.wa = q.wa; f.wb = q.wb; f.lds_bytes = (uint32_t)lds;
    f.rw_a = q.a.rw; f.rw_b = q.b.rw;
    return true;
}

#endif

template <int GS, int B>
static hipError_t launch_b(const GemvArgs &a, const Q80GemvPlan &p, hipStream_t st) {
    GemvDev d = to_dev(a);
    if (p.kernel == Q80_KERNEL_STREAM) return launch_stream_b<GS, B>(d, p, st);
    d.tile_max = nullptr;
    return launch_slab_b<GS, B>(d, p, st);
}
template <int GS>
static hipError_t launch_gs(const GemvArgs &a, const Q80GemvPlan &p, hipStream_t st) {
    if (p.gs != (uint32_t)GS) return hipErrorInvalidValue;
    if (p.B == 1) return launch_b<GS, 1>(a, p, st);
    if (p.B == 2) return launch_b<GS, 2>(a, p, st);
    if (p.B == 4) return launch_b<GS, 4>(a, p, st);
    return launch_b<GS, 8>(a, p, st);
}

}

hipError_t NANO_Q80_ENTRY(const GemvArgs &a, const Q80GemvPlan &p, hipStream_t st) { return launch_gs<NANO_Q80_GS>(a, p, st); }

#if NANO_Q80_GS == 64
bool qkv_attn_fused_q80_plan(const GemvArgs &ga, const AttnArgs &aa, QkvAttnFusedPlan *out) {
    QkvAttnFusedPlan f;
    if (!fused_shape(ga, aa, f)) return false;
    if (out) *out = f;
    return true;
}

hipError_t launch_qkv_attn_fused_q80(const GemvArgs &ga, const AttnArgs &aa, unsigned long long *hand, uint32_t *tick, uint32_t layer1, hipStream_t st) {
    QkvAttnFusedPlan p;
    if (!hand || !tick || !layer1 || layer1 > 127u || !fused_shape(ga, aa, p)) return hipErrorInvalidValue;
    GemvDev d = to_dev(ga);
    d.tile_max = nullptr;
    d.rw = p.rw; d.tpw = (p.rw + 3) / 4; d.magic_rw = 65536u / p.rw + 1u; d.log2_tiles = 0;
    d.units = d.tpw * d.nchunk;
    d.wg_c0 = p.wg[0]; d.wg_c1 = p.wg[0] + p.wg[1];
    d.nthr = p.threads;
    QkvAttnArgs fa{};
    fused_attn_setup(fa, aa, hand, tick, layer1);
    const uint32_t grid = p.n_attn + p.ngemv;
    const size_t lds = p.lds_bytes;
    fa.g = d; fa.ngemv = p.ngemv;
    fa.wait16 = 1u;
    if (p.kernel == FUSED_KERNEL_Q80_WF) { hipLaunchKernelGGL(qkv_attn_fused_wf_kernel, dim3(grid), dim3(p.threads), lds, st, fa); return hipGetLastError(); }
#define FUSED_GO(NV_, UPW_) do { if (p.nv == NV_ && p.upw == UPW_) { hipLaunchKernelGGL((qkv_attn_fused_kernel<NV_, UPW_>), dim3(grid), dim3(p.threads), lds, st, fa); return hipGetLastError(); } } while (0)
    FUSED_GO(1, 1); FUSED_GO(1, 2); FUSED_GO(1, 4);
    FUSED_GO(2, 1); FUSED_GO(2, 2);
#undef FUSED_GO
    return hipErrorInvalidValue;
}

bool wo_w13_fused_plan(const GemvArgs &wo, const GemvArgs &w13, WoW13FusedPlan *out) {
    WoW13FusedPlan f; GemvDev da, db;
    if (!wo13_shape(wo, w13, f, da, db)) return false;
    if (out) *out = f;
    return true;
}

hipError_t launch_wo_w13_fused(const GemvArgs &wo, const GemvArgs &w13, unsigned long long *hand, uint32_t *tick, uint32_t layer1, hipStream_t st) {
    WoW13FusedPlan q;
    Wo13Args fa{};
    if (!hand || !tick || !layer1 || layer1 > 127u || !wo13_shape(wo, w13, q, fa.wo, fa.w13)) return hipErrorInvalidValue;
    fa.wo_wgs = q.wa;
    fa.wait16 = 4u;
    SlabHand h{};
    h.buf = hand; h.tick = tick; h.layer1 = layer1;
    h.base[0] = 0; h.base[1] = 0; h.base[2] = 0;
    fa.hand = h;
    const size_t lds = q.lds_bytes;
#define WO13_GO(RA_, WF_, WFC_) do { if (q.role == (uint32_t)RA_ && q.wf == WF_ && q.wfc == WFC_) { \
        hipLaunchKernelGGL((wo_w13_fused_kernel<RA_, WF_, WFC_>), dim3(q.wb), dim3(q.threads), lds, st, fa); return hipGetLastError(); } } while (0)
    WO13_GO(R_RESID, 0, 0); WO13_GO(R_RESID, 0, 2); WO13_GO(R_RESID, 1, 0); WO13_GO(R_RESID, 1, 2);
    WO13_GO(R_RESID_COMBINE, 0, 0); WO13_GO(R_RESID_COMBINE, 0, 2); WO13_GO(R_RESID_COMBINE, 1, 0); WO13_GO(R_RESID_COMBINE, 1, 2);
#undef WO13_GO
    return hipErrorInvalidValue;
}
#endif

}
```

### nano_amd/csrc/gemv_q80_slab_body.inc

```
#ifndef SLAB_WF
#define SLAB_WF 0
#define SLAB_WF_DEFAULTED 1
#endif
#ifndef SLAB_WFC
#define SLAB_WFC 0
#define SLAB_WFC_DEFAULTED 1
#endif
#ifndef SLAB_EARLY
#define SLAB_EARLY 0
#define SLAB_EARLY_DEFAULTED 1
#endif
#ifndef SLAB_XHAND_WAIT
#define SLAB_XHAND_WAIT 0u
#define SLAB_XHAND_NAP 0
#define SLAB_XHAND_WAIT_DEFAULTED 1
#endif
#define SLAB_ISSUE_UNIT(k) do { \
      if constexpr (WFPAIR_) { \
         \
         \
        const uint32_t u = (uint32_t)wid + (uint32_t)k * NW; \
        const bool live = u < SLAB_A.units; \
        const __amdgpu_buffer_rsrc_t rw0_ = mkrsrc(w0, live ? rows0 * n : 0u), rw1_ = mkrsrc(SLAB_A.w[1], live ? rows0 * n : 0u); \
        const __amdgpu_buffer_rsrc_t rs0_ = mkrsrc(ws0, live ? rows0 * ng * 4u : 0u), rs1_ = mkrsrc(SLAB_A.ws[1], live ? rows0 * ng * 4u : 0u); \
        const uint32_t lrow = lrow0 + u * 2u, base = lrow * n + (uint32_t)lane * 16u; \
        _Pragma("unroll") \
        for (int r = 0; r < TR; r++) wv[k][r] = bload_w(r < 2 ? rw0_ : rw1_, (u * 2u + (uint32_t)(r & 1) < RW) ? base + (uint32_t)(r & 1) * n : OOB); \
        const uint32_t r_ = (uint32_t)lane & 3u, rr_ = r_ & 1u; \
        const uint32_t so_ = (u * 2u + rr_ < RW) ? ((lrow + rr_) * ng + ((uint32_t)lane >> 2)) * 4u : OOB; \
        const float s0_ = bload_f(rs0_, r_ < 2u ? so_ : OOB), s1_ = bload_f(rs1_, r_ < 2u ? OOB : so_); \
        sv[k][0] = __uint_as_float(__float_as_uint(s0_) | __float_as_uint(s1_)); \
      } else { \
        const uint32_t u = (uint32_t)wid + (uint32_t)k * NW; \
        const uint32_t t = (u * SLAB_A.magic_nchunk) >> 16; \
        const uint32_t c = u - t * SLAB_A.nchunk; \
        const uint32_t mat = t >= TPW ? 1u : 0u, tl = t - mat * TPW; \
        const bool live = u < SLAB_A.units; \
        const __amdgpu_buffer_rsrc_t rw_ = mkrsrc(mat ? SLAB_A.w[1] : w0, live ? rows0 * n : 0u); \
        const __amdgpu_buffer_rsrc_t rs_ = mkrsrc(mat ? SLAB_A.ws[1] : ws0, live ? rows0 * ng * 4u : 0u); \
        const uint32_t lrow = lrow0 + tl * TR; \
        const uint32_t col = (c << 10) + (uint32_t)lane * 16u; \
        const uint32_t base = (col < n) ? lrow * n + col : OOB; \
        _Pragma("unroll") \
        for (int r = 0; r < TR; r++) wv[k][r] = bload_w(rw_, base + ((tl * TR + (uint32_t)r < RW) ? (uint32_t)r * n : OOB)); \
        const uint32_t g = c * GC + (uint32_t)lane / LPG; \
        _Pragma("unroll") \
        for (int s = 0; s < NS; s++) { \
            const uint32_t r = ((uint32_t)lane % LPG) + s * LPG; \
            sv[k][s] = bload_f(rs_, (r < TR && tl * TR + r < RW && g < ng) ? ((lrow + r) * ng + g) * 4u : OOB); \
        } \
      } \
    } while (0)
#if SLAB_PART != 2
    constexpr int TR = 4;
    constexpr int LPG = GS / 16, GC = 1024 / GS;
    constexpr int NS = (TR + LPG - 1) / LPG;
    const int tid = threadIdx.x, lane = tid & 63;
    const int wid = __builtin_amdgcn_readfirstlane(tid >> 6);
    const int NW = (int)(SLAB_A.nthr >> 6);
    constexpr bool WF_ = (SLAB_WF) != 0, WFPAIR_ = WF_ && ROLE == R_NORM_SWIGLU;
    static_assert(!WF_ || (GS == 64 && B == 1 && (SLAB_EARLY) == 0 && (ROLE == R_NORM_STORE || ROLE == R_NORM_SWIGLU)), "SLAB_WF: one-chunk rows of the rmsnorm roles");
    constexpr int NCH_ = (SLAB_WFC);
    constexpr bool WFC_ = NCH_ != 0;
    constexpr uint32_t UP_ = NCH_ <= 2 ? 4u : 8u;
    static_assert(!WFC_ || (!WF_ && NCH_ >= 2 && NCH_ <= 4 && GS == 64 && B == 1 && (SLAB_EARLY) == 0 && (ROLE == R_RESID || ROLE == R_RESID_COMBINE)), "SLAB_WFC: whole-chunk rows of the residual roles");
    const uint32_t n = WF_ ? 1024u : WFC_ ? (uint32_t)NCH_ * 1024u : SLAB_A.n, ng = WF_ ? 16u : WFC_ ? (uint32_t)NCH_ * 16u : SLAB_A.ng;
    const uint32_t n16 = (n + 15) & ~15u, ng4 = (ng + 3) & ~3u;
    const uint32_t PITCH = (GC == 16) ? (((ng + 47) / 64) * 64 + 16) : (ng4 + 4);
    const uint32_t RW = SLAB_A.rw, TPW = SLAB_A.tpw, RWP = TPW * TR;
    const uint32_t epi = role_epi<ROLE>(SLAB_A);
    const bool swiglu = epi == GEMV_EPI_SWIGLU;
    const uint32_t nmat = swiglu ? 2 : 1;
    int8_t *xq = reinterpret_cast<int8_t *>(smem);
    float *xs = reinterpret_cast<float *>(smem + B * n16);
    float *red = xs + B * ng4;
    float *P = red + B * 16 + (has_flag<ROLE>(SLAB_A, F_COMBINE) ? B * SLAB_A.attn_n_head * 8 : 0);

    karg_touch(SLAB_A.out[0]); karg_touch(SLAB_A.out_bstride[0]); karg_touch(SLAB_A.out_pstride[0]); karg_touch(SLAB_A.rows[0]); karg_touch(SLAB_A.magic_rw); karg_touch(SLAB_A.nb);
    if (!(ROLE == R_RESID || ROLE == R_RESID_COMBINE || ROLE == R_NORM_SWIGLU)) {
        karg_touch(SLAB_A.out[1]); karg_touch(SLAB_A.out[2]); karg_touch(SLAB_A.out_bstride[1]); karg_touch(SLAB_A.out_bstride[2]);
        karg_touch(SLAB_A.out_pstride[1]); karg_touch(SLAB_A.out_pstride[2]); karg_touch(SLAB_A.rows[1]); karg_touch(SLAB_A.rows[2]);
    }
    karg_touch(SLAB_A.pos); karg_touch(SLAB_A.canon);
    if (ROLE == R_GENERIC || ROLE == R_RESID || ROLE == R_RESID_COMBINE) { karg_touch(SLAB_A.resid_add); karg_touch(SLAB_A.resid_add_bstride); }
    NANO_STAMP(SLAB_A.stamps, 0, tid);
    Staged<B, NV> sx;
    if constexpr (SLAB_XHAND) stage_issue_nw<ROLE, B, NV>(SLAB_A, sx);
    else if (!(NANO_STAMPS && (SLAB_A.dbg & 2u))) stage_issue<ROLE, B, NV>(SLAB_A, sx);

    constexpr bool ONESEG = ROLE == R_RESID || ROLE == R_RESID_COMBINE || ROLE == R_NORM_SWIGLU;
    const int sel = (ONESEG || swiglu) ? 0 : (int)(SLAB_BID >= SLAB_A.wg_c0) + (int)(SLAB_BID >= SLAB_A.wg_c1);
    const int8_t *w0 = sel == 0 ? SLAB_A.w[0] : sel == 1 ? SLAB_A.w[1] : SLAB_A.w[2];
    const float *ws0 = sel == 0 ? SLAB_A.ws[0] : sel == 1 ? SLAB_A.ws[1] : SLAB_A.ws[2];
    float *out0 = sel == 0 ? SLAB_A.out[0] : sel == 1 ? SLAB_A.out[1] : SLAB_A.out[2];
    const uint32_t rows0 = sel == 0 ? SLAB_A.rows[0] : sel == 1 ? SLAB_A.rows[1] : SLAB_A.rows[2];
    const uint32_t obs = sel == 0 ? SLAB_A.out_bstride[0] : sel == 1 ? SLAB_A.out_bstride[1] : SLAB_A.out_bstride[2];
    const uint32_t ops = sel == 0 ? SLAB_A.out_pstride[0] : sel == 1 ? SLAB_A.out_pstride[1] : SLAB_A.out_pstride[2];
    const uint32_t lrow0 = (SLAB_BID - (sel == 0 ? 0u : sel == 1 ? SLAB_A.wg_c0 : SLAB_A.wg_c1)) * RW;

    int4 wv[UPW][TR];
    float sv[UPW][NS];
    constexpr uint32_t early_ = (uint32_t)(SLAB_EARLY);
    static_assert(SLAB_PART == 0 || early_ == 0u, "SLAB_EARLY: the whole body only");
#pragma unroll
    for (int k = 0; k < UPW; k++) { if (early_ == 0u || (uint32_t)k < early_) SLAB_ISSUE_UNIT(k); }
    if (!SLAB_XHAND && NANO_STAMPS && (SLAB_A.dbg & 2u)) stage_issue<ROLE, B, NV>(SLAB_A, sx);
    const int fb = (int)(((uint32_t)tid * SLAB_A.magic_rw) >> 16);
    const int frl = tid - fb * (int)RW;
    const bool fold_live = tid < (int)(RW * B) && fb < (int)SLAB_A.nb && lrow0 + frl < rows0;
    uint32_t opos = 0;
    if constexpr (WF_) {
        if constexpr (ROLE == R_NORM_STORE) opos = __float_as_uint(bload_f(mkrsrc(SLAB_A.pos, ops ? 4u : 0u), ((uint32_t)lane & ~3u) == (uint32_t)WF_LANE0 ? 0u : OOB));
    } else
    if (ops && fold_live) opos = SLAB_A.pos[fb];
    float oldv = 0.0f;
    if (epi == GEMV_EPI_RESID && fold_live) oldv = out0[(size_t)fb * obs + lrow0 + frl];
    float addv = 0.0f;
    const bool has_add = epi == GEMV_EPI_RESID && SLAB_A.resid_add != nullptr;
    if (has_add && fold_live) addv = SLAB_A.resid_add[(size_t)fb * SLAB_A.resid_add_bstride + lrow0 + frl];

    NANO_STAMP(SLAB_A.stamps, 1, oldv);
#endif
#if SLAB_PART != 1
    if constexpr (SLAB_XHAND) {
        static_assert(!SLAB_XHAND || B == 1, "granule activations: one sequence");
        const unsigned long long *hb_ = SLAB_XHANDV.buf;
        const uint32_t ctag_ = SLAB_CTAG;
        bool got_ = false;
        for (uint32_t w_ = 0; w_ < SLAB_XHAND_WAIT; w_++) __builtin_amdgcn_s_sleep(16);
        for (uint32_t spin_ = 0; spin_ < (1u << 14) && !got_; spin_++) {
            if (spin_) __builtin_amdgcn_s_sleep(SLAB_XHAND_NAP);
            if ((spin_ & 63u) == 63u && hand_aborted(SLAB_XHANDV)) break;
            got_ = true;
#pragma unroll
            for (int j = 0; j < NV; j++) {
                const uint32_t i = ((uint32_t)tid + (uint32_t)j * SLAB_A.nthr) * 4u;
                if (i < n) {
                    const unsigned long long g0_ = __hip_atomic_load(hb_ + i, __ATOMIC_RELAXED, __HIP_MEMORY_SCOPE_AGENT);
                    const unsigned long long g1_ = __hip_atomic_load(hb_ + i + 1, __ATOMIC_RELAXED, __HIP_MEMORY_SCOPE_AGENT);
                    const unsigned long long g2_ = __hip_atomic_load(hb_ + i + 2, __ATOMIC_RELAXED, __HIP_MEMORY_SCOPE_AGENT);
                    const unsigned long long g3_ = __hip_atomic_load(hb_ + i + 3, __ATOMIC_RELAXED, __HIP_MEMORY_SCOPE_AGENT);
                    got_ = got_ && (uint32_t)(g0_ >> 32) == ctag_ && (uint32_t)(g1_ >> 32) == ctag_ && (uint32_t)(g2_ >> 32) == ctag_ && (uint32_t)(g3_ >> 32) == ctag_;
                    sx.x[0][j] = make_float4(__uint_as_float((uint32_t)g0_), __uint_as_float((uint32_t)g1_), __uint_as_float((uint32_t)g2_), __uint_as_float((uint32_t)g3_));
                } else sx.x[0][j] = make_float4(0.f, 0.f, 0.f, 0.f);
            }
        }
        if (!got_) hand_give_up(SLAB_XHANDV, SLAB_A.err);
    }
    stage_finish<ROLE, GS, B, NV>(SLAB_A, sx, xq, xs, red, n16, ng4);
    if constexpr (early_ != 0u) {
#pragma unroll
        for (int k = 1; k < UPW; k++) { if ((uint32_t)k >= early_) SLAB_ISSUE_UNIT(k); }
    }
    NANO_STAMP(SLAB_A.stamps, 3, xs[0]);

    if constexpr (WF_) {
    float pw_[UPW];
    const int4 xv_ = *reinterpret_cast<const int4 *>(xq + lane * 16);
    const float xsc_ = xs[lane >> 2];
    asm volatile("" :: "v"(xsc_));
#pragma unroll
    for (int k = 0; k < UPW; k++) {
        int iv[TR];
#pragma unroll
        for (int r = 0; r < TR; r++) {
            int d = __builtin_amdgcn_sdot4(wv[k][r].x, xv_.x, 0, false);
            d = __builtin_amdgcn_sdot4(wv[k][r].y, xv_.y, d, false);
            d = __builtin_amdgcn_sdot4(wv[k][r].z, xv_.z, d, false);
            d = __builtin_amdgcn_sdot4(wv[k][r].w, xv_.w, d, false);
            iv[r] = dpp_group_sum<LPG>(d);
        }
        int v = iv[0];
#pragma unroll
        for (int q = 1; q < TR; q++) v = (q == (lane & 3)) ? iv[q] : v;
        pw_[k] = ((float)v * sv[k][0]) * xsc_;
    }
    NANO_STAMP(SLAB_A.stamps, 4, pw_[UPW - 1]);
    NANO_STAMP(SLAB_A.stamps, 5, pw_[UPW - 1]);
#pragma unroll
    for (int k = 0; k < UPW; k++) {
        const uint32_t u = (uint32_t)wid + (uint32_t)k * NW;
        if (u < SLAB_A.units) {
            const float v0 = wave_fold_canon16(pw_[k]);
            const float v1 = WFPAIR_ ? DPP_F(v0, 0x102) : 0.0f;
            const uint32_t rl_ = WFPAIR_ ? u * 2u + ((uint32_t)lane & 1u) : u * (uint32_t)TR + ((uint32_t)lane & 3u);
            const bool mine_ = WFPAIR_ ? ((uint32_t)lane & ~1u) == (uint32_t)WF_LANE0 : ((uint32_t)lane & ~3u) == (uint32_t)WF_LANE0;
            if (mine_ && rl_ < RW && lrow0 + rl_ < rows0) {
                float *dst = out0 + (size_t)opos * ops + lrow0 + rl_;
                const float val = finish_epi(epi, v0, v1, 0.0f);
                if constexpr (SLAB_HAND == 1)
                    __hip_atomic_store(SLAB_HANDV.buf + (sel == 0 ? SLAB_HANDV.base[0] : sel == 1 ? SLAB_HANDV.base[1] : SLAB_HANDV.base[2]) + lrow0 + rl_,
                                       ((unsigned long long)(SLAB_PTAG) << 32) | (unsigned long long)__float_as_uint(val), __ATOMIC_RELAXED, __HIP_MEMORY_SCOPE_AGENT);
                if (NANO_STAMPS && (SLAB_A.dbg & 4u)) *dst = val; else __hip_atomic_store(dst, val, __ATOMIC_RELAXED, __HIP_MEMORY_SCOPE_AGENT);
            }
        }
    }
    } else {
#pragma unroll
    for (int k = 0; k < UPW; k++) {
        const uint32_t u = (uint32_t)wid + (uint32_t)k * NW;
        if (u < SLAB_A.units) {
            const uint32_t t = (u * SLAB_A.magic_nchunk) >> 16;
// ... 108 lines not shown
                for (int q = 0; q < 4; q++) { v0 += t[q].x; v0 += t[q].y; v0 += t[q].z; v0 += t[q].w; }
                if (swiglu) {
#pragma unroll
                    for (int q = 0; q < 4; q++) { v1 += u[q].x; v1 += u[q].y; v1 += u[q].z; v1 += u[q].w; }
                }
            }
        } else {
        for (uint32_t g0 = 0; g0 < ng; g0 += 16) {
                float4 t[4], u[4];
#pragma unroll
                for (int q = 0; q < 4; q++) {
                    t[q] = (g0 + 4 * q < ng4) ? *reinterpret_cast<const float4 *>(p0 + g0 + 4 * q) : make_float4(0.f, 0.f, 0.f, 0.f);
                    if (swiglu) u[q] = (g0 + 4 * q < ng4) ? *reinterpret_cast<const float4 *>(p1 + g0 + 4 * q) : make_float4(0.f, 0.f, 0.f, 0.f);
                }
#pragma unroll
                for (int q = 0; q < 4; q++) {
                    const uint32_t g = g0 + 4 * q;
                    v0 += (g < ng) ? t[q].x : 0.0f; v0 += (g + 1 < ng) ? t[q].y : 0.0f; v0 += (g + 2 < ng) ? t[q].z : 0.0f; v0 += (g + 3 < ng) ? t[q].w : 0.0f;
                }
                if (swiglu) {
#pragma unroll
                    for (int q = 0; q < 4; q++) {
                        const uint32_t g = g0 + 4 * q;
                        v1 += (g < ng) ? u[q].x : 0.0f; v1 += (g + 1 < ng) ? u[q].y : 0.0f; v1 += (g + 2 < ng) ? u[q].z : 0.0f; v1 += (g + 3 < ng) ? u[q].w : 0.0f;
                    }
                }
            }
        }
        if (fold_live) {
            float *dst = out0 + (size_t)fb * obs + (size_t)opos * ops + lrow0 + frl;
            const float val = finish_epi(epi, has_add ? v0 + addv : v0, v1, oldv);
            if constexpr (SLAB_HAND == 1)
                __hip_atomic_store(SLAB_HANDV.buf + (sel == 0 ? SLAB_HANDV.base[0] : sel == 1 ? SLAB_HANDV.base[1] : SLAB_HANDV.base[2]) + lrow0 + (uint32_t)frl,
                                   ((unsigned long long)(SLAB_PTAG) << 32) | (unsigned long long)__float_as_uint(val), __ATOMIC_RELAXED, __HIP_MEMORY_SCOPE_AGENT);
            if (NANO_STAMPS && (SLAB_A.dbg & 4u)) *dst = val; else __hip_atomic_store(dst, val, __ATOMIC_RELAXED, __HIP_MEMORY_SCOPE_AGENT);
        }
    }
    }
    NANO_STAMP_END(SLAB_A.stamps, 6);
#endif
#undef SLAB_ISSUE_UNIT
#ifdef SLAB_WF_DEFAULTED
#undef SLAB_WF
#undef SLAB_WF_DEFAULTED
#endif
#ifdef SLAB_WFC_DEFAULTED
#undef SLAB_WFC
#undef SLAB_WFC_DEFAULTED
#endif
#ifdef SLAB_EARLY_DEFAULTED
#undef SLAB_EARLY
#undef SLAB_EARLY_DEFAULTED
#endif
#ifdef SLAB_XHAND_WAIT_DEFAULTED
#undef SLAB_XHAND_WAIT
#undef SLAB_XHAND_NAP
#undef SLAB_XHAND_WAIT_DEFAULTED
#endif
```

### nano_amd/csrc/kernels.h

```cpp
#pragma once

#include <hip/hip_runtime.h>
#include <stddef.h>
#include <stdint.h>
#include "../../include/nano_mi355x.h"
#include "device_common.h"

namespace nano {

enum : uint32_t { GEMV_EPI_STORE = 0, GEMV_EPI_RESID = 1, GEMV_EPI_SWIGLU = 2 };

struct GemvSeg {
    const void *w;
    const float *ws;
    float *out;
    uint32_t rows;
    uint32_t out_bstride;
    uint32_t out_pstride;
    uint32_t _pad;
};

struct GemvArgs {
    GemvSeg seg[3];
    uint32_t nseg;
    uint32_t n;
    uint32_t gs;
    uint32_t nb;
    const float *xin;
    uint32_t xin_bstride;
    uint32_t epi;
    const float *norm_w;
    const uint32_t *pos;
    uint32_t tiles;
    uint32_t frag_ready;
    const int8_t *xq_in;
    const float *xs_in;
    const uint8_t *x4_in;
    uint8_t *q4_scratch; size_t q4_scratch_bytes;
    float *f32_scratch; size_t f32_scratch_floats;
    const float *attn_part;
    const float *attn_ml;
    uint32_t attn_nsplit, attn_n_head, attn_hd, _pad2;
    const float *resid_add; uint32_t resid_add_bstride, _pad3;
    float *tile_max;
    uint32_t cus;
    uint32_t ordered;
    uint32_t *err;
    unsigned long long *stamps;
};


inline bool q80_canonical(const GemvArgs &a) {
    if (a.ordered || a.gs != 64 || a.n % 256u) return false;
    if (a.nseg == 1 && a.epi == GEMV_EPI_STORE && a.seg[0].rows >= 16384u && a.seg[0].out_pstride == 0) return false;
    return true;
}
uint32_t gemv_tiles(uint32_t quant, const GemvArgs &a);
hipError_t launch_gemv(uint32_t quant, GemvArgs &a, hipStream_t st);
inline uint32_t gemv_total_rows(const GemvArgs &a) {
    if (a.epi == GEMV_EPI_SWIGLU) return a.seg[0].rows;
    uint32_t r = 0;
    for (uint32_t s = 0; s < a.nseg; s++) r += a.seg[s].rows;
    return r;
}
hipError_t launch_gemv_q4k(const GemvArgs &a, hipStream_t st);
constexpr uint32_t GEMV_Q4K_LDS_MAX = 160 * 1024;
constexpr uint32_t GEMV_Q4K_CHUNK_SEARCH_LDS = 150 * 1024;
enum : uint32_t { Q4K_KERNEL_NONE = 0, Q4K_KERNEL_SLAB = 1, Q4K_KERNEL_CHUNK = 2 };
struct Q4kGemvPlan {
    uint32_t kernel, role, B;
    uint32_t nv, ipt;
    uint32_t d, loop, rounds, wg[3];
    uint32_t rw, nthr, grid, lds_bytes;
    uint32_t pre;
    uint32_t quant_rows, quant_nthr, quant_nv;
    uint32_t partials;
};
bool gemv_q4k_plan(const GemvArgs &a, Q4kGemvPlan *p);
uint32_t gemv_q4k_fit_batch(const GemvArgs &a);
bool gemm_q4k_supports(const GemvArgs &a);
hipError_t launch_gemm_q4k(const GemvArgs &a, hipStream_t st);
hipError_t launch_gemv_q80(const GemvArgs &a, hipStream_t st);
hipError_t launch_gemv_f32(const GemvArgs &a, hipStream_t st);
constexpr uint32_t GEMV_Q80_LDS_MAX = 160 * 1024;
enum : uint32_t { Q80_KERNEL_NONE = 0, Q80_KERNEL_SLAB = 1, Q80_KERNEL_STREAM = 2 };
enum : uint32_t { Q80_VAR_PLAIN = 0, Q80_VAR_EARLY = 1, Q80_VAR_WF = 2, Q80_VAR_WFC2 = 3, Q80_VAR_WFC3 = 4, Q80_VAR_WFC4 = 5 };
struct Q80GemvPlan {
    uint32_t kernel, role, gs, B, nv, upw;
    uint32_t rw, nw, grid, lds_bytes;
    uint32_t variant, pre;
    uint32_t early, units, wg_c0, wg_c1;
};
bool gemv_q80_plan(const GemvArgs &a, Q80GemvPlan *p);
uint32_t gemv_q80_fit_batch(const GemvArgs &a);
constexpr uint32_t GEMV_F32_LDS_MAX = 160 * 1024;
struct F32GemvPlan { uint32_t role, B, nv, upw, rw, nw, grid, lds_bytes; };
bool gemv_f32_plan(const GemvArgs &a, F32GemvPlan *p);
uint32_t gemv_f32_fit_batch(const GemvArgs &a);
constexpr uint32_t GEMM_F32_LDS_MAX = 160 * 1024;
struct F32GemmPlan {
    uint32_t sw;
    uint32_t threads, grid, lds_bytes;
    uint32_t rt, nw, nt, nu, upw, tp;
    uint32_t stage_bytes, tab_off;
    uint32_t pro_threads, pro_lds;
    uint32_t xs_floats;
};
bool gemm_f32_plan(const GemvArgs &a, F32GemmPlan *p);
inline bool gemm_f32_supports(const GemvArgs &a) { return gemm_f32_plan(a, nullptr); }
hipError_t launch_gemm_f32(const GemvArgs &a, hipStream_t st);
enum : uint32_t { Q80_GEMM_NONE, Q80_GEMM_G6S, Q80_GEMM_G6F, Q80_GEMM_G7, Q80_GEMM_G7K, Q80_GEMM_GC, Q80_GEMM_G2 };
struct Q80GemmPlan {
    uint32_t kernel;
    uint32_t tt, nv, r, ms, tp, pp, gs, sw;
    uint32_t threads, grid, lds_bytes;
    uint32_t norm_order;
    uint32_t hh, ntiles, tc0, tc1, tpw, full, nu, nk, ttl;
    uint32_t nw, rounds, tts;
    uint32_t magic;
    uint32_t nsa, pre, a_stage, a_ws, b_base, b_stage, b_xs;
    uint32_t ks, ncw, nss, tab, ring, nl;
    uint32_t waves, lt, nhc, nwaves;
    uint32_t ng, npass;
};
bool gemm_q80_plan(const GemvArgs &a, Q80GemmPlan *p);
hipError_t launch_quant_rows_frag(const float *x, uint32_t x_bstride, const float *norm_w, uint32_t n, uint32_t gs, uint32_t nb,
                                  int8_t *xf, float *xsf, hipStream_t st, uint32_t order = 256);
hipError_t launch_quant_rows(const float *x, uint32_t x_bstride, const float *norm_w, uint32_t n, uint32_t gs, uint32_t nb,
                             int8_t *xq, float *xs, hipStream_t st);
uint32_t gemv_q80_partials(const GemvArgs &a);

enum RouteKind : uint32_t {
    ROUTE_GEMV = 0,
    ROUTE_GEMV_PREQ,
    ROUTE_GEMV_SLICED,
    ROUTE_Q4K,
    ROUTE_RESERVED,
    ROUTE_FRAG_G6,
    ROUTE_FRAG_OLD,
    ROUTE_FRAG_G7,
    ROUTE_Q4K_GEMM,
    ROUTE_F32_GEMM,
};
inline bool route_takes_fragments(RouteKind k) { return k == ROUTE_FRAG_G6 || k == ROUTE_FRAG_OLD || k == ROUTE_FRAG_G7; }
// ... 24 lines not shown
    float *q_out;
    const float *kraw;
    float *kcache;
    float *vcache;
    const uint32_t *pos;
    const float *q_norm;
    const float *k_norm;
    const float *rope_cos;
    const float *rope_sin;
    const float *rope_cur;
    float *out;
    float *ml;
    float *xba_out;
    uint32_t nsplit;
    uint32_t range_hint;
    uint32_t layer, n_layer, S, hd, n_head, n_kv_head, q_dim, kv_dim;
    uint32_t rope_qwen3;
    uint32_t is_causal;
    uint32_t cache_bstride_rows;
    uint32_t fixed_range;
    uint32_t prep_only;
    uint32_t kv_half;
    const float *vraw;
    int8_t *xf_out; float *xsf_out;
    uint32_t kv_log2, kvmul_log2;
    const uint32_t *pt_rows;
    const uint32_t *kvrow;
    uint32_t pt_stride, pt_bstride;
    uint32_t pool_rows, _pad6;
    uint32_t *err;
    unsigned long long *stamps;
    const uint32_t *row_slot;
};
hipError_t launch_attention(const AttnArgs &a, uint32_t nb, hipStream_t st);
struct AttnPlan { uint32_t mode, lpr, qv, kvm, npt, w16, paged, kv_half, nsplit, kv_log2, kvmul_log2; };
bool attention_plan(const AttnArgs &a, uint32_t nb, AttnPlan *p);
hipError_t launch_attention_fp8(const AttnArgs &a, const AttnPlan &p, uint32_t nb, hipStream_t st);
enum : uint32_t { FUSED_KERNEL_NONE = 0, FUSED_KERNEL_Q80_TABLE = 1, FUSED_KERNEL_Q80_WF = 2, FUSED_KERNEL_Q4K = 3, FUSED_KERNEL_F32 = 4 };
constexpr uint32_t FUSED_LDS_MAX = 64 * 1024;
struct QkvAttnFusedPlan {
    uint32_t kernel, nv;
    uint32_t upw, d, qv;
    uint32_t threads, n_attn, ngemv, lds_bytes;
    uint32_t rw, wg[3], rounds;
};
bool qkv_attn_fused_plan(uint32_t quant, const GemvArgs &ga, const AttnArgs &aa, QkvAttnFusedPlan *p);
inline bool qkv_attn_fused_supports(uint32_t quant, const GemvArgs &ga, const AttnArgs &aa) { return qkv_attn_fused_plan(quant, ga, aa, nullptr); }
hipError_t launch_qkv_attn_fused(uint32_t quant, const GemvArgs &ga, const AttnArgs &aa, unsigned long long *hand, uint32_t *tick, uint32_t layer1, hipStream_t st);
struct WoW13FusedPlan {
    uint32_t sig, threads, role, wf, wfc;
    uint32_t nv_a, upw_a, nv_b, upw_b;
    uint32_t wa, wb, lds_bytes;
    uint32_t rw_a, rw_b;
};
bool wo_w13_fused_plan(const GemvArgs &wo, const GemvArgs &w13, WoW13FusedPlan *p);
inline bool wo_w13_fused_supports(const GemvArgs &wo, const GemvArgs &w13) { return wo_w13_fused_plan(wo, w13, nullptr); }
hipError_t launch_wo_w13_fused(const GemvArgs &wo, const GemvArgs &w13, unsigned long long *hand, uint32_t *tick, uint32_t layer1, hipStream_t st);
inline bool fused_attn_side_ok(const AttnArgs &aa, uint32_t qr, uint32_t kr, uint32_t vr, bool plain) {
    if (plain ? (aa.hd < 4u || aa.hd > 64u || aa.hd % 4u || aa.q_norm || aa.k_norm || aa.rope_qwen3) : (aa.hd != 128u || !aa.q_norm || !aa.k_norm || !aa.rope_qwen3)) return false;
    if (!aa.rope_cos || !aa.rope_cur || !aa.kraw || aa.fixed_range || !aa.is_causal || aa.q_out) return false;
    if (aa.kv_half || aa.pt_rows || aa.prep_only || aa.xf_out || aa.nsplit == 0 || aa.nsplit > 8u) return false;
    const uint32_t kv_mul = aa.n_kv_head ? aa.n_head / aa.n_kv_head : 0u;
    if (!aa.n_kv_head || (aa.n_kv_head & (aa.n_kv_head - 1u)) || !kv_mul || (kv_mul & (kv_mul - 1u))) return false;
    if ((uint64_t)aa.n_head * aa.nsplit > 256u) return false;
    if (aa.range_hint > aa.nsplit * 2u * 32u) return false;
    return aa.q_dim == qr && aa.kv_dim == kr && aa.kv_dim == vr && aa.q_dim == aa.n_head * aa.hd;
}
hipError_t handoff_alloc(uint32_t **tick, unsigned long long **hand, size_t granules, unsigned long long **hand2, size_t granules2);
uint32_t attention_nsplit(uint32_t range_hint, uint32_t hd);
hipError_t launch_attn_combine(const float *part, const float *ml, float *out, uint32_t n_head, uint32_t hd, uint32_t nsplit, hipStream_t st);
hipError_t launch_attn_combine_tokens(const float *part, const float *ml, float *out, uint32_t n_head, uint32_t hd, uint32_t nsplit, uint32_t nb,
                                      int8_t *xf_out, float *xsf_out, hipStream_t st);

struct StrictAttnArgs {
    float *q;
    const float *kraw;
    float *kcache, *vcache;
    const uint32_t *pos;
    const float *q_norm, *k_norm;
    const float *rope_cos, *rope_sin;
    float *att;
    float *xba;
    uint32_t n_head, n_kv_head, hd, q_dim, kv_dim, layer, n_layer, S;
    uint32_t slot0;
    uint32_t rope_qwen3, is_causal;
    uint32_t fold_prep;
};
hipError_t launch_strict_rmsnorm(float *o, const float *x, const float *w, uint32_t n, uint32_t nvec, uint32_t x_stride, uint32_t o_stride, hipStream_t st);
hipError_t launch_strict_qk(const StrictAttnArgs &a, uint32_t nb, hipStream_t st);
hipError_t launch_strict_attention(const StrictAttnArgs &a, uint32_t nb, hipStream_t st);
hipError_t launch_strict_swiglu(float *hb, const float *hb2, uint32_t n, uint32_t nb, uint32_t bstride, hipStream_t st);
hipError_t launch_strict_matmul_f32(float *out, const float *x, const float *w, uint32_t n, uint32_t d, uint32_t nb, uint32_t x_bstride,
                                    uint32_t out_bstride, uint32_t out_pstride, const uint32_t *pos, int resid, hipStream_t st);

hipError_t launch_exact_rmsnorm(float *o, const float *x, const float *w, uint32_t n, uint32_t nvec, uint32_t x_stride, uint32_t o_stride, hipStream_t st);
bool exact_attention_fits(uint32_t hd, uint32_t max_range);
hipError_t launch_exact_attention(const StrictAttnArgs &a, uint32_t nb, hipStream_t st);

const char *lora_shape_error(uint32_t E, uint32_t rank);
struct LoraSlotDesc {
    const float *t[8];
    uint32_t rank, alpha;
};
struct LoraRowsArgs {
    const LoraSlotDesc *desc;
    const float *x;
// ... 188 lines not shown
```

### nano_amd/csrc/ops.hip

```cpp
#include <stdio.h>
#include <string.h>

#include <algorithm>
#include <array>
#include <string>
#include <vector>

#include "../../include/nano_mi355x.h"
#include "kernels.h"
#include "pool_plan.h"

using namespace nano;

extern "C" const char *nano_hip_last_error(void);
namespace { thread_local std::string g_op_err; }

extern "C" void nano_hip_set_error_(const char *msg);

struct DevBufs {
    std::vector<void *> ptrs;
    ~DevBufs() { for (void *p : ptrs) (void)hipFree(p); }
    template <typename T> T *alloc(size_t n) {
        void *p = nullptr;
        if (hipMalloc(&p, n * sizeof(T) + 16) != hipSuccess) return nullptr;
// ... 290 lines not shown
    if (p->max_draft > LOOKUP_MAX_ROWS - 1 || dn > n - 1) { nano_hip_set_error_("draft_round: max_draft beyond 15, or dn beyond n - 1"); return NANO_HIP_EINVAL; }
    int rc; if ((rc = begin(device))) return rc;
    DevBufs B;
    DraftArgs a{};
    const uint32_t room = n + LOOKUP_MAX_ROWS, full = seq_limit < room ? seq_limit + 1u : room;
    a.cap = ((full > n ? full : n) + 3u) & ~3u;
    a.hist = B.alloc<uint32_t>(a.cap > room ? a.cap : room);
    const uint32_t st[4] = { n, left, 0u, 0u };
    a.state = B.upload(st, 4);
    uint32_t *toks = B.alloc<uint32_t>(LOOKUP_MAX_ROWS);
    a.fed = toks; a.amax = nb ? B.upload(amax, nb) : nullptr; a.ids = nb > 1 ? B.upload(fed + 1, nb - 1) : nullptr; a.nb = nb;
    a.max_draft = p->max_draft; a.stop_token = p->stop_token; a.seq_limit = seq_limit; a.dn = dn;
    a.next_tokens = toks; a.next_pos = B.alloc<uint32_t>(LOOKUP_MAX_ROWS); a.record = B.alloc<uint32_t>(DRAFT_REC_WORDS);
    OP_CHECK(a.hist && a.state && toks && (!nb || a.amax) && (nb < 2 || a.ids) && a.next_pos && a.record, "device alloc failed");
    OP_HIP(hipMemset(a.hist, 0xff, (size_t)(a.cap > room ? a.cap : room) * 4));
    OP_HIP(hipMemcpy(a.hist, history, (size_t)n * 4, hipMemcpyHostToDevice));
    OP_HIP(hipMemset(toks, 0xff, LOOKUP_MAX_ROWS * 4)); OP_HIP(hipMemset(a.next_pos, 0xff, LOOKUP_MAX_ROWS * 4));
    if (nb) OP_HIP(hipMemcpy(toks, fed, 4, hipMemcpyHostToDevice));
    if (nb > 1) { a.role = DRAFT_ROLE_STAGE; OP_HIP(launch_draft_round(a, 0)); }
    a.role = DRAFT_ROLE_ACCEPT;
    OP_HIP(launch_draft_round(a, 0));
    OP_HIP(hipMemcpy(record_out, a.record, DRAFT_REC_WORDS * 4, hipMemcpyDeviceToHost));
    OP_HIP(hipMemcpy(history, a.hist, (size_t)room * 4, hipMemcpyDeviceToHost));
    OP_HIP(hipMemcpy(next_tokens_out, toks, LOOKUP_MAX_ROWS * 4, hipMemcpyDeviceToHost));
    OP_HIP(hipMemcpy(next_pos_out, a.next_pos, LOOKUP_MAX_ROWS * 4, hipMemcpyDeviceToHost));
    return 0;
}

static const char *fused_desc_shape_error(const NanoFusedGemvDesc &d) {
    if (d.kind > 2 || d.nseg == 0 || d.nseg > 3 || (d.kind == 2 && d.nseg != 2) || d.nb == 0 || d.nb > NANO_MAX_BATCH || d.n % 4) return "bad fused-gemv descriptor";
    if (d.quant == NANO_QUANT_Q80 && (!(d.gs == 32 || d.gs == 64 || d.gs == 128 || d.gs == 256) || d.n % d.gs || d.n % 16)) return "bad n / group size";
    for (uint32_t s = 0; s < d.nseg; s++) if (!d.rows[s]) return "missing weight tensor";
    if (d.kind == 2 && d.rows[0] != d.rows[1]) return "W1 / W3 row counts differ";
    if (d.resid_add && (d.kind != 1 || d.resid_add_stride < d.rows[0])) return "bad residual addend";
    if (d.attn_part && (!d.attn_nsplit || d.attn_nsplit > 8 || !d.attn_n_head || d.attn_n_head * d.attn_hd != d.n || d.kind != 1 || (d.nb > 8 && d.quant != NANO_QUANT_Q4K))) return "bad attention partials";
    return nullptr;
}

enum F32Scratch { F32X_NONE, F32X_ASKED, F32X_MODEL };
struct FusedLaunch {
    GemvArgs a;
    Q80Route r;
    size_t gq_bytes, gxs_floats;
};
static FusedLaunch fused_launch(const NanoFusedGemvDesc &d, uint32_t cus, F32Scratch f32x) {
    FusedLaunch L{};
    GemvArgs &a = L.a;
    Q80Route &r = L.r;
    for (uint32_t s = 0; s < d.nseg; s++) a.seg[s].rows = d.rows[s];
    a.nseg = d.nseg; a.n = d.n; a.gs = d.gs; a.nb = d.nb; a.cus = cus ? cus : 256u;
    a.epi = d.kind == 0 ? GEMV_EPI_STORE : d.kind == 1 ? GEMV_EPI_RESID : GEMV_EPI_SWIGLU;
    a.norm_w = d.norm_w;
    if (d.attn_part) { a.attn_part = d.attn_part; a.attn_nsplit = d.attn_nsplit; a.attn_n_head = d.attn_n_head; a.attn_hd = d.attn_hd; }
    if (d.resid_add) { a.resid_add = d.resid_add; a.resid_add_bstride = d.resid_add_stride; }
    a.ordered = d.ordered ? 1u : 0u;
    r.quant = d.quant; r.cus = (int)a.cus; r.mfma_min_nb = (d.use_gemm && d.quant == NANO_QUANT_Q80) ? 1u : 9u;
    if (d.quant == NANO_QUANT_Q80) {
        const size_t n16 = (d.n + 15) & ~(size_t)15, tiles = (d.nb + 15) / 16, tt = tiles > 2 ? 4 : tiles;
        L.gq_bytes = tt * 16 * n16; L.gxs_floats = tt * 16 * (d.n / d.gs);
    }
    if (d.quant == NANO_QUANT_Q4K && d.nb > 1) r.q4x_bytes = (size_t)(d.nb > 8 ? d.nb : 8u) * ((d.n + 255) & ~(size_t)255);
    if (d.quant == NANO_QUANT_F32 && (f32x == F32X_MODEL || (f32x == F32X_ASKED && d.use_gemm && d.nb > 8))) {
        r.f32_min_nb = 9u;
        r.f32x_floats = f32x == F32X_MODEL ? ~(size_t)0 : (size_t)((d.nb + 15) / 16) * 16 * ((d.n + 127) & ~(size_t)127);
    }
    return L;
}
alignas(8) static uint8_t g_flag[8];
static void flag_scratch(FusedLaunch &L) {
    uint8_t *const flag = g_flag;
    if (L.gq_bytes) L.r.gq = reinterpret_cast<int8_t *>(flag);
    if (L.gxs_floats) L.r.gxs = reinterpret_cast<float *>(flag);
    if (L.r.q4x_bytes) L.r.q4x = flag;
    if (L.r.f32x_floats) L.r.f32x = reinterpret_cast<float *>(flag);
}
static int query_begin(const NanoFusedGemvDesc *dp, uint32_t cus, uint32_t *out, uint32_t words, uint32_t quant, const char *not_quant,
                       F32Scratch f32x, FusedLaunch *L) {
    if (!dp || !out) { nano_hip_set_error_("null argument"); return NANO_HIP_EINVAL; }
    if (dp->quant != quant) { nano_hip_set_error_(not_quant); return NANO_HIP_EINVAL; }
    if (const char *msg = fused_desc_shape_error(*dp)) { nano_hip_set_error_(msg); return NANO_HIP_EINVAL; }
    memset(out, 0, words * sizeof(uint32_t));
    *L = fused_launch(*dp, cus, f32x);
    flag_scratch(*L);
    return 0;
}
template <uint32_t WORDS, typename Plan, typename Fields>
static int report_first_slice(FusedLaunch &L, uint32_t *out, bool (*plan)(const GemvArgs &, Plan *), Fields fields) {
    GemvArgs &a = L.a;
    uint32_t per = 0, launches = 0;
    Plan p;
    if (!route_gemv_slices(L.r.quant, a, &per, &launches)) return 0;
    a.nb = per;
    if (launches > 1) a.tile_max = nullptr;
    if (!plan(a, &p)) return 0;
    const auto v = fields(p);
    static_assert(std::tuple_size<decltype(v)>::value + 3 <= WORDS, "the plan's fields and the three words of the slicing fit the query's output");
    memcpy(out, v.data(), sizeof(v));
    const uint32_t tail[3] = { launches, per, 1u };
    memcpy(out + v.size(), tail, sizeof(tail));
    return 0;
}
template <size_t N> using Words = std::array<uint32_t, N>;

extern "C" int nano_hip_f32_gemv_plan(const NanoFusedGemvDesc *dp, uint32_t cus, uint32_t out[NANO_F32_GEMV_PLAN_WORDS]) {
    FusedLaunch L;
    if (int rc = query_begin(dp, cus, out, NANO_F32_GEMV_PLAN_WORDS, NANO_QUANT_F32, "not an FP32 launch", F32X_NONE, &L)) return rc;
    return report_first_slice<NANO_F32_GEMV_PLAN_WORDS>(L, out, gemv_f32_plan, [](const F32GemvPlan &p) {
        return Words<8>{{ p.role, p.B, p.nv, p.upw, p.rw, p.nw, p.grid, p.lds_bytes }}; });
}

extern "C" int nano_hip_f32_gemm_plan(const NanoFusedGemvDesc *dp, uint32_t cus, uint32_t out[NANO_F32_GEMM_PLAN_WORDS]) {
    static_assert(sizeof(F32GemmPlan) == (NANO_F32_GEMM_PLAN_WORDS - 2) * sizeof(uint32_t), "the query reports every field of the plan");
    FusedLaunch L;
    if (int rc = query_begin(dp, cus, out, NANO_F32_GEMM_PLAN_WORDS, NANO_QUANT_F32, "not an FP32 launch", F32X_MODEL, &L)) return rc;
    const RouteKind k = route_kind(L.r, L.a);
    out[0] = (uint32_t)k;
    F32GemmPlan p{};
    if (k == ROUTE_F32_GEMM && gemm_f32_plan(L.a, &p)) memcpy(out + 1, &p, sizeof(p));
    out[NANO_F32_GEMM_PLAN_WORDS - 1] = 1u;
    return 0;
}

extern "C" int nano_hip_q80_gemv_plan(const NanoFusedGemvDesc *dp, uint32_t cus, uint32_t out[NANO_Q80_GEMV_PLAN_WORDS]) {
    FusedLaunch L;
    if (int rc = query_begin(dp, cus, out, NANO_Q80_GEMV_PLAN_WORDS, NANO_QUANT_Q80, "not a Q80 launch", F32X_NONE, &L)) return rc;
    GemvArgs &a = L.a;
    const uint32_t k = (uint32_t)route_kind(L.r, a);
    if (route_takes_fragments((RouteKind)k)) {
        out[0] = k; out[13] = 1u; out[14] = a.nb; out[15] = 1u;
        return 0;
    }
    if (k == ROUTE_GEMV_PREQ) { a.xq_in = L.r.gq; a.xs_in = L.r.gxs; a.norm_w = nullptr; }
    return report_first_slice<NANO_Q80_GEMV_PLAN_WORDS>(L, out, gemv_q80_plan, [k](const Q80GemvPlan &p) {
        return Words<13>{{ k, p.kernel, p.role, p.gs, p.B, p.nv, p.upw, p.rw, p.nw, p.grid, p.lds_bytes, p.variant, p.pre }}; });
}

extern "C" int nano_hip_q80_gemm_plan(const NanoFusedGemvDesc *dp, uint32_t cus, uint32_t out[NANO_Q80_GEMM_PLAN_WORDS]) {
    static_assert(sizeof(Q80GemmPlan) == (NANO_Q80_GEMM_PLAN_WORDS - 2) * sizeof(uint32_t), "the query reports every field of the plan");
    FusedLaunch L;
    if (int rc = query_begin(dp, cus, out, NANO_Q80_GEMM_PLAN_WORDS, NANO_QUANT_Q80, "not a Q80 launch", F32X_NONE, &L)) return rc;
    Q80GemmPlan p{};
    out[0] = (uint32_t)route_kind(L.r, L.a, &p);
    memcpy(out + 1, &p, sizeof(p));
    out[NANO_Q80_GEMM_PLAN_WORDS - 1] = 1u;
    return 0;
}

extern "C" int nano_hip_q4k_gemv_plan(const NanoFusedGemvDesc *dp, uint32_t cus, uint32_t out[NANO_Q4K_GEMV_PLAN_WORDS]) {
    static float asked;
    FusedLaunch L;
    if (int rc = query_begin(dp, cus, out, NANO_Q4K_GEMV_PLAN_WORDS, NANO_QUANT_Q4K, "not a Q4K launch", F32X_NONE, &L)) return rc;
    GemvArgs &a = L.a;
    if (a.epi == GEMV_EPI_STORE && a.nseg == 1) a.tile_max = &asked;
    const uint32_t k = (uint32_t)route_kind(L.r, a);
    if (k == ROUTE_Q4K_GEMM) {
        out[0] = k; out[21] = 1u; out[22] = a.nb; out[23] = 1u;
        return 0;
    }
    route_fill(L.r, a);
    return report_first_slice<NANO_Q4K_GEMV_PLAN_WORDS>(L, out, gemv_q4k_plan, [k](const Q4kGemvPlan &p) {
        return Words<21>{{ k, p.kernel, p.role, p.B, p.nv, p.ipt, p.d, p.loop, p.rounds, p.wg[0], p.wg[1], p.wg[2], p.rw, p.nthr, p.grid,
                           p.lds_bytes, p.pre, p.quant_rows, p.quant_nthr, p.quant_nv, p.partials }}; });
}

static int upload_weights(DevBufs &B, const NanoFusedGemvDesc &d, GemvArgs &a) {
    const size_t bpl = (d.n + 255) / 256;
    for (uint32_t s = 0; s < d.nseg; s++) {
        const size_t rows = d.rows[s];
        if (!d.w[s]) { nano_hip_set_error_("missing weight tensor"); return NANO_HIP_EINVAL; }
        if (d.quant == NANO_QUANT_Q80) {
            a.seg[s].w = B.upload(reinterpret_cast<const int8_t *>(d.w[s]), rows * d.n);
            a.seg[s].ws = B.upload(d.ws[s], rows * d.n / d.gs);
            OP_CHECK(a.seg[s].ws, "device alloc failed");
        } else if (d.quant == NANO_QUANT_Q4K) a.seg[s].w = B.upload(reinterpret_cast<const uint8_t *>(d.w[s]), rows * bpl * 160);
        else a.seg[s].w = B.upload(reinterpret_cast<const float *>(d.w[s]), rows * d.n);
        OP_CHECK(a.seg[s].w, "device alloc failed");
    }
    return 0;
}

extern "C" int nano_hip_op_fused_gemv(int device, const NanoFusedGemvDesc *dp) {
    int rc; if ((rc = begin(device))) return rc;
    if (!dp) { nano_hip_set_error_("null descriptor"); return NANO_HIP_EINVAL; }
    const NanoFusedGemvDesc &d = *dp;
    if (!d.out) { nano_hip_set_error_("bad fused-gemv descriptor"); return NANO_HIP_EINVAL; }
    if (!d.x && !d.attn_part) { nano_hip_set_error_("no activation"); return NANO_HIP_EINVAL; }
// ... 244 lines not shown
        memcpy(row, v, sizeof(v));
        return true;
    };
    if (d.chunk) {
        a.prep_only = 1;
        OP_ARG(record(a, plan[0]), "attention arguments refused");
        OP_HIP(launch_attention(a, nb, 0));
        a.prep_only = 0;
    }
    OP_ARG(record(a, plan[d.chunk ? 1 : 0]), "attention arguments refused");
    OP_HIP(launch_attention(a, nb, 0));
    if (nsplit > 1) OP_HIP(launch_attn_combine_tokens(dpart, dml, dout, d.n_head, d.hd, nsplit, nb, nullptr, nullptr, 0));
    OP_HIP(hipDeviceSynchronize());
    OP_HIP(hipMemcpy(d.out, dout, (size_t)nb * QD * 4, hipMemcpyDeviceToHost));
    OP_HIP(hipMemcpy(d.k_cache, dkc, cache_elems * esz, hipMemcpyDeviceToHost));
    OP_HIP(hipMemcpy(d.v_cache, dvc, cache_elems * esz, hipMemcpyDeviceToHost));
    if (d.want_frag) {
        OP_HIP(hipMemcpy(d.xf, a.xf_out, ntile * ng * 1024, hipMemcpyDeviceToHost));
        OP_HIP(hipMemcpy(d.xsf, a.xsf_out, ntile * ng * 16 * 4, hipMemcpyDeviceToHost));
    }
    if (d.plan) memcpy(d.plan, plan, sizeof(plan));
#undef OP_ARG
    return 0;
}

static bool qkv_attn_fused_resolve(const NanoFusedGemvDesc &g, const NanoAttnDecodeDesc &ad, uint32_t cus, FusedLaunch &L, AttnArgs &a, QkvAttnFusedPlan &p) {
    if (fused_desc_shape_error(g) || g.kind != 0 || g.nb != 1 || ad.nb != 1 || ad.chunk || ad.want_frag) return false;
    if (!ad.n_head || !ad.n_kv_head || ad.n_head % ad.n_kv_head || !ad.hd || !ad.range_hint) return false;
    L = fused_launch(g, cus, F32X_MODEL);
    flag_scratch(L);
    route_fill(L.r, L.a);
    a = attn_launch(ad, attn_desc_nsplit(ad));
    const float *flag = reinterpret_cast<const float *>(g_flag);
    a.kraw = flag; a.rope_cos = flag; a.rope_sin = flag; a.rope_cur = flag;
    if (ad.pool_rows) a.pt_rows = reinterpret_cast<const uint32_t *>(g_flag);
    if (route_kind(L.r, L.a) != (g.quant == NANO_QUANT_Q4K ? ROUTE_Q4K : ROUTE_GEMV)) return false;
    return qkv_attn_fused_plan(g.quant, L.a, a, &p);
}
static bool wo_w13_fused_resolve(const NanoFusedGemvDesc &wo, const NanoFusedGemvDesc &w13, uint32_t cus, FusedLaunch &La, FusedLaunch &Lb, WoW13FusedPlan &p) {
    if (fused_desc_shape_error(wo) || fused_desc_shape_error(w13) || wo.quant != NANO_QUANT_Q80 || w13.quant != NANO_QUANT_Q80) return false;
    if (wo.kind != 1 || w13.kind != 2 || wo.nb != 1 || w13.nb != 1 || wo.nseg != 1) return false;
    La = fused_launch(wo, cus, F32X_NONE); Lb = fused_launch(w13, cus, F32X_NONE);
    flag_scratch(La); flag_scratch(Lb);
    route_fill(La.r, La.a); route_fill(Lb.r, Lb.a);
    La.a.seg[0].out = reinterpret_cast<float *>(g_flag); Lb.a.xin = La.a.seg[0].out;
    if (route_kind(La.r, La.a) != ROUTE_GEMV || route_kind(Lb.r, Lb.a) != ROUTE_GEMV) return false;
    return wo_w13_fused_plan(La.a, Lb.a, &p);
}
static void plan_words(const QkvAttnFusedPlan &p, uint32_t *out) {
    const uint32_t v[NANO_QKV_ATTN_FUSED_PLAN_WORDS] = { p.kernel, p.nv, p.upw, p.d, p.qv, p.threads, p.n_attn, p.ngemv, p.lds_bytes, p.rw, p.wg[0], p.wg[1], p.wg[2], p.rounds, 0u, 1u };
    memcpy(out, v, sizeof(v));
}
static void plan_words(const WoW13FusedPlan &p, uint32_t *out) {
    const uint32_t v[NANO_WO_W13_FUSED_PLAN_WORDS] = { p.sig, p.threads, p.role, p.wf, p.wfc, p.nv_a, p.upw_a, p.nv_b, p.upw_b, p.wa, p.wb, p.lds_bytes, p.rw_a, p.rw_b, 0u, 1u };
    memcpy(out, v, sizeof(v));
}

extern "C" int nano_hip_qkv_attn_fused_plan(const NanoFusedGemvDesc *qkv, const NanoAttnDecodeDesc *attn, uint32_t cus, uint32_t out[NANO_QKV_ATTN_FUSED_PLAN_WORDS]) {
    if (!qkv || !attn || !out) { nano_hip_set_error_("null argument"); return NANO_HIP_EINVAL; }
    memset(out, 0, NANO_QKV_ATTN_FUSED_PLAN_WORDS * sizeof(uint32_t));
    FusedLaunch L; AttnArgs a; QkvAttnFusedPlan p;
    if (qkv_attn_fused_resolve(*qkv, *attn, cus, L, a, p)) plan_words(p, out);
    return 0;
}
extern "C" int nano_hip_wo_w13_fused_plan(const NanoFusedGemvDesc *wo, const NanoFusedGemvDesc *w13, uint32_t cus, uint32_t out[NANO_WO_W13_FUSED_PLAN_WORDS]) {
    if (!wo || !w13 || !out) { nano_hip_set_error_("null argument"); return NANO_HIP_EINVAL; }
    memset(out, 0, NANO_WO_W13_FUSED_PLAN_WORDS * sizeof(uint32_t));
    FusedLaunch La, Lb; WoW13FusedPlan p;
    if (wo_w13_fused_resolve(*wo, *w13, cus, La, Lb, p)) plan_words(p, out);
    return 0;
}

struct HandoffState {
    uint32_t *tick = nullptr; unsigned long long *hand = nullptr;
    uint32_t *h_err = nullptr, *dev_err = nullptr;
    ~HandoffState() { (void)hipFree(tick); (void)hipFree(hand); if (h_err) (void)hipHostFree(h_err); }
    int init(size_t granules, const unsigned long long *hand_init, uint32_t tick0) {
        OP_HIP(handoff_alloc(&tick, &hand, granules, nullptr, 0));
        if (hand_init) OP_HIP(hipMemcpy(hand, hand_init, granules * 8, hipMemcpyHostToDevice));
        const uint32_t t = tick0 + 1u;
        OP_HIP(hipMemcpy(tick, &t, 4, hipMemcpyHostToDevice));
        OP_HIP(hipHostMalloc(reinterpret_cast<void **>(&h_err), 64, hipHostMallocMapped));
        *h_err = 0;
        OP_HIP(hipHostGetDevicePointer(reinterpret_cast<void **>(&dev_err), h_err, 0));
        return 0;
    }
    int finish(uint32_t *err_out) {
        const uint32_t c = *reinterpret_cast<volatile uint32_t *>(h_err);
        if (err_out) *err_out = c;
        if (c & NANO_DEVERR_HANDOFF) { nano_hip_set_error_("a consumer of the fused launch gave up waiting for its producers: no result is valid"); return NANO_HIP_ERUNTIME; }
        return 0;
    }
};
#define OP_ARG(cond, msg) do { if (!(cond)) { nano_hip_set_error_(msg); return NANO_HIP_EINVAL; } } while (0)

extern "C" int nano_hip_op_qkv_attn_fused(int device, const NanoQkvAttnFusedDesc *dp) {
    int rc; if ((rc = begin(device))) return rc;
    OP_ARG(dp && dp->qkv && dp->attn, "null descriptor");
    const NanoFusedGemvDesc &g = *dp->qkv;
    const NanoAttnDecodeDesc &d = *dp->attn;
    OP_ARG(dp->layer1 >= 1 && dp->layer1 <= 127, "layer1 outside 1 .. 127");
    if (const char *msg = fused_desc_shape_error(g)) { nano_hip_set_error_(msg); return NANO_HIP_EINVAL; }
    OP_ARG(g.x && g.norm_w, "the projection needs x and norm_w");
    OP_ARG(d.nb == 1 && d.n_layer && d.layer < d.n_layer && d.S, "bad nb / layer / S");
    OP_ARG(d.pos && d.rope_cos && d.rope_sin && d.k_cache && d.v_cache && d.out, "missing tensor");
    OP_ARG(!d.q_norm == !d.k_norm, "q_norm and k_norm go together");
    OP_ARG(d.range_hint >= d.pos[0] + 1 && d.range_hint <= d.S, "range_hint must cover pos + 1 and stay <= S");
// ... 102 lines not shown
```

Before: 2052.

## Combine split-attention partials per wave in registers inside Wo GEMV

Adds a combine-wave path for the single-sequence Wo projection that merges split-KV attention partials. Each wave loads the partial outputs and (m,l) stats into registers, reduces the softmax weights with DPP and broadcasts them with ds_bpermute, then forms the combined input without the LDS weight table or its block barrier. New CW variants of the slab kernel and the fused Wo/W13 kernel are instantiated and used by default, with an env var to fall back to the table path. The register path holds up to eight partial vectors per thread, which raises register pressure, and it only covers head dims that are powers of two from 32 to 256 with at most eight splits.

```diff
diff --git a/include/nano_mi355x.h b/include/nano_mi355x.h
--- a/include/nano_mi355x.h
+++ b/include/nano_mi355x.h
@@ -371,7 +371,7 @@
 int nano_hip_f32_gemv_plan(const NanoFusedGemvDesc *d, uint32_t cus, uint32_t out[NANO_F32_GEMV_PLAN_WORDS]);
 #define NANO_F32_GEMM_PLAN_WORDS 17
 int nano_hip_f32_gemm_plan(const NanoFusedGemvDesc *d, uint32_t cus, uint32_t out[NANO_F32_GEMM_PLAN_WORDS]);
-#define NANO_Q80_GEMV_PLAN_WORDS 16
+#define NANO_Q80_GEMV_PLAN_WORDS 17
 int nano_hip_q80_gemv_plan(const NanoFusedGemvDesc *d, uint32_t cus, uint32_t out[NANO_Q80_GEMV_PLAN_WORDS]);
 #define NANO_Q80_GEMM_PLAN_WORDS 47
 int nano_hip_q80_gemm_plan(const NanoFusedGemvDesc *d, uint32_t cus, uint32_t out[NANO_Q80_GEMM_PLAN_WORDS]);
@@ -379,7 +379,7 @@
 int nano_hip_q4k_gemv_plan(const NanoFusedGemvDesc *d, uint32_t cus, uint32_t out[NANO_Q4K_GEMV_PLAN_WORDS]);
 
 #define NANO_QKV_ATTN_FUSED_PLAN_WORDS 16
-#define NANO_WO_W13_FUSED_PLAN_WORDS 16
+#define NANO_WO_W13_FUSED_PLAN_WORDS 17
 int nano_hip_qkv_attn_fused_plan(const NanoFusedGemvDesc *qkv, const NanoAttnDecodeDesc *attn, uint32_t cus, uint32_t out[NANO_QKV_ATTN_FUSED_PLAN_WORDS]);
 int nano_hip_wo_w13_fused_plan(const NanoFusedGemvDesc *wo, const NanoFusedGemvDesc *w13, uint32_t cus, uint32_t out[NANO_WO_W13_FUSED_PLAN_WORDS]);
 typedef struct NanoQkvAttnFusedDesc {
diff --git a/nano_amd/binding.py b/nano_amd/binding.py
--- a/nano_amd/binding.py
+++ b/nano_amd/binding.py
@@ -87,6 +87,7 @@
 
 Q80_PLAN_FIELDS = ("route", "kernel", "role", "gs", "B", "nv", "upw", "rw", "nw", "grid", "lds_bytes", "variant", "pre", "launches",
                    "seqs_per_launch", "takes")
+Q80_PLAN_WORDS = len(Q80_PLAN_FIELDS) + 1
 Q80_ROLES = F32_ROLES
 Q80_KERNELS = ("none", "slab", "stream")
 Q80_VARIANTS = ("plain", "early", "wf", "wfc2", "wfc3", "wfc4")
@@ -107,7 +108,7 @@
 QKV_ATTN_FUSED_PLAN_FIELDS = ("kernel", "nv", "upw", "d", "qv", "threads", "n_attn", "ngemv", "lds_bytes", "rw", "wg0", "wg1", "wg2", "rounds",
                               "_zero", "takes")
 WO_W13_FUSED_PLAN_FIELDS = ("sig", "threads", "role", "wf", "wfc", "nv_a", "upw_a", "nv_b", "upw_b", "wa", "wb", "lds_bytes", "rw_a", "rw_b",
-                            "_zero", "takes")
+                            "_zero", "takes", "cw")
 FUSED_KERNELS = ("none", "q80_table", "q80_wf", "q4k", "f32")
 NANO_DEVERR_HANDOFF = 2
 
@@ -901,7 +902,12 @@
 
 def q80_gemv_plan(kind, n, rows, nb=1, *, gs=64, norm=False, attn=None, ordered=False, use_gemm=False, resid_add=False, cus=256):
     d = _fused_shape(0x80, kind, n, rows, nb, gs=gs, norm=bool(norm), attn=attn, ordered=ordered, use_gemm=use_gemm, resid_add=bool(resid_add))
-    return _plan_query("q80_gemv", Q80_PLAN_FIELDS, len(Q80_PLAN_FIELDS), d, cus)
+    return _plan_query("q80_gemv", Q80_PLAN_FIELDS, Q80_PLAN_WORDS, d, cus)
+
+
+def q80_gemv_plan_cw(kind, n, rows, nb=1, *, gs=64, norm=False, attn=None, ordered=False, use_gemm=False, resid_add=False, cus=256):
+    d = _fused_shape(0x80, kind, n, rows, nb, gs=gs, norm=bool(norm), attn=attn, ordered=ordered, use_gemm=use_gemm, resid_add=bool(resid_add))
+    return _plan_query("q80_gemv", Q80_PLAN_FIELDS + ("cw",), Q80_PLAN_WORDS, d, cus)["cw"]
 
 
 def q80_gemm_plan(kind, n, rows, nb=1, *, gs=64, norm=False, attn=None, ordered=False, use_gemm=False, cus=256):
diff --git a/nano_amd/csrc/backend.hip b/nano_amd/csrc/backend.hip
--- a/nano_amd/csrc/backend.hip
+++ b/nano_amd/csrc/backend.hip
@@ -305,6 +305,7 @@
     if (getenv("NANO_HIP_NO_GRAPH")) m->use_graph = false;
     if (const char *nt = getenv("NANO_KV_COPY_NT")) m->kv.copy_nt = *nt && *nt != '0';
     if (const char *fz = getenv("NANO_FUSE_LAUNCHES")) { const uint32_t v = (uint32_t)strtoul(fz, nullptr, 0); m->ho.fuse_qkv_attn = (v & 1u) != 0; m->ho.fuse_wo_w13 = (v & 2u) != 0; }
+    if (const char *cwv = getenv("NANO_COMBINE_WAVE")) m->ho.combine_wave = *cwv != '0';
     {
         const bool gran = (m->d.quant_type == NANO_QUANT_Q80 && m->d.group_size == 64) || m->d.quant_type == NANO_QUANT_Q4K || m->d.quant_type == NANO_QUANT_F32;
         const size_t g1 = gran ? (size_t)m->QD + 2 * (size_t)m->KD : 0, g2 = (gran && m->d.quant_type == NANO_QUANT_Q80) ? (size_t)m->d.n_embd : 0;
diff --git a/nano_amd/csrc/backend_model.h b/nano_amd/csrc/backend_model.h
--- a/nano_amd/csrc/backend_model.h
+++ b/nano_amd/csrc/backend_model.h
@@ -129,6 +129,7 @@
         unsigned long long *hand = nullptr;
         bool fuse_wo_w13 = true;
         unsigned long long *hand2 = nullptr;
+        bool combine_wave = true;
         uint32_t *tick = nullptr;
         uint32_t fallbacks = 0;
         bool reissue = true;
diff --git a/nano_amd/csrc/backend_step.hip b/nano_amd/csrc/backend_step.hip
--- a/nano_amd/csrc/backend_step.hip
+++ b/nano_amd/csrc/backend_step.hip
@@ -74,7 +74,7 @@
     GemvArgs a = proj_args(m, nb, m->QD, m->xba, GEMV_EPI_RESID);
     a.nseg = 1; a.seg[0] = mkseg(m->W[WO][l], m->x, m->d.n_embd, m->d.n_embd);
     if (m->lora_on) { a.resid_add = m->lora_o1; a.resid_add_bstride = m->d.n_embd; }
-    if (nsplit > 1) { a.attn_part = m->attn_part; a.attn_ml = m->attn_ml; a.attn_nsplit = nsplit; a.attn_n_head = m->d.n_head; a.attn_hd = m->hd; }
+    if (nsplit > 1) { a.attn_part = m->attn_part; a.attn_ml = m->attn_ml; a.attn_nsplit = nsplit; a.attn_n_head = m->d.n_head; a.attn_hd = m->hd; a.attn_table = m->ho.combine_wave ? 0u : 1u; }
     return a;
 }
 static GemvArgs w13_args(const NanoHipModel *m, uint32_t l, uint32_t nb, const float *xin, const float *norm_w, float *w3_out, uint32_t epi) {
diff --git a/nano_amd/csrc/gemv_common.h b/nano_amd/csrc/gemv_common.h
--- a/nano_amd/csrc/gemv_common.h
+++ b/nano_amd/csrc/gemv_common.h
@@ -114,13 +114,91 @@
     float4 nw[NV];
     float4 pv[B == 1 ? NV : 1][B == 1 ? 8 : 1];
     float ml_m, ml_l;
+    float cw_m[B == 1 ? NV : 1], cw_l[B == 1 ? NV : 1];
 };
 template <int B>
 struct Staged<B, 0> {};
 
-template <int ROLE, int B, int NV>
+template <int NV, int S>
+__device__ __forceinline__ void cw_issue_from(const GemvDev &a, const __amdgpu_buffer_rsrc_t rp, Staged<1, NV> &r) {
+    if constexpr (S < 8) {
+        if (S == 0 || a.attn_nsplit > (uint32_t)S) {
+#pragma unroll
+            for (int j = 0; j < NV; j++) {
+                const uint32_t i = (threadIdx.x + (uint32_t)j * a.nthr) * 4u;
+                r.pv[j][S] = bload_f4(rp, (i < a.n) ? ((uint32_t)S * a.n + i) * 4u : OOB);
+            }
+            cw_issue_from<NV, S + 1>(a, rp, r);
+        }
+    }
+}
+template <int NV>
+__device__ __forceinline__ void cw_issue(const GemvDev &a, Staged<1, NV> &r) {
+    const uint32_t ns = a.attn_nsplit, nh = a.attn_n_head, n = a.n;
+    const uint32_t lane = threadIdx.x & 63u, wid = threadIdx.x >> 6, NW = a.nthr >> 6;
+    cw_issue_from<NV, 0>(a, mkrsrc(a.attn_part, ns * n * 4u), r);
+    const __amdgpu_buffer_rsrc_t rm = mkrsrc(a.attn_ml, nh * ns * 8u);
+    const uint32_t hpw = 256u >> (uint32_t)__builtin_ctz(a.attn_hd), sp = lane & 7u, hl = lane >> 3;
+#pragma unroll
+    for (int j = 0; j < NV; j++) {
+        const uint32_t h = (wid + (uint32_t)j * NW) * hpw + hl;
+        const uint32_t mo = (hl < hpw && sp < ns) ? ((h < nh ? h : 0u) * ns + sp) * 8u : OOB;
+        r.cw_m[j] = bload_f(rm, mo);
+        r.cw_l[j] = bload_f(rm, mo == OOB ? OOB : mo + 4u);
+    }
+}
+__device__ __forceinline__ float cw_mad(float acc, float p, float w) {
+    float t, r;
+    asm("v_mul_f32_e32 %0, %1, %2" : "=v"(t) : "v"(p), "v"(w));
+    asm("v_add_f32_e32 %0, %1, %2" : "=v"(r) : "v"(acc), "v"(t));
+    return r;
+}
+template <int NV, int S>
+__device__ __forceinline__ void cw_add_from(const GemvDev &a, const Staged<1, NV> &r, const float (&w)[NV][8], float4 (&acc)[NV]) {
+    if constexpr (S < 8) {
+        if (S == 0 || a.attn_nsplit > (uint32_t)S) {
+#pragma unroll
+            for (int j = 0; j < NV; j++) {
+                acc[j].x = cw_mad(acc[j].x, r.pv[j][S].x, w[j][S]); acc[j].y = cw_mad(acc[j].y, r.pv[j][S].y, w[j][S]);
+                acc[j].z = cw_mad(acc[j].z, r.pv[j][S].z, w[j][S]); acc[j].w = cw_mad(acc[j].w, r.pv[j][S].w, w[j][S]);
+            }
+            cw_add_from<NV, S + 1>(a, r, w, acc);
+        }
+    }
+}
+template <int NV>
+__device__ __forceinline__ void cw_combine(const GemvDev &a, Staged<1, NV> &r) {
+    const uint32_t lane = threadIdx.x & 63u;
+    const int src = (int)((((lane * 4u) >> (uint32_t)__builtin_ctz(a.attn_hd)) * 8u) * 4u);
+    float w[NV][8];
+#pragma unroll
+    for (int j = 0; j < NV; j++) {
+        const float m = r.cw_m[j], l = r.cw_l[j];
+        const bool live = l > 0.0f;
+        float M = live ? m : -INFINITY;
+        M = fmaxf(M, DPP_F(M, 0xB1)); M = fmaxf(M, DPP_F(M, 0x4E)); M = fmaxf(M, DPP_F(M, 0x141));
+        const float e = live ? expf(m - M) : 0.0f;
+        float L = l * e;
+        L += DPP_F(L, 0xB1); L += DPP_F(L, 0x4E); L += DPP_F(L, 0x141);
+        const int wq = __float_as_int(e / L);
+#pragma unroll
+        for (int s = 0; s < 8; s++) w[j][s] = __int_as_float(__builtin_amdgcn_ds_bpermute(src + 4 * s, wq));
+    }
+    float4 acc[NV];
+#pragma unroll
+    for (int j = 0; j < NV; j++) acc[j] = make_float4(0.f, 0.f, 0.f, 0.f);
+    cw_add_from<NV, 0>(a, r, w, acc);
+#pragma unroll
+    for (int j = 0; j < NV; j++) r.x[0][j] = acc[j];
+}
+
+template <int ROLE, int B, int NV, int CW = 0>
 __device__ __forceinline__ void stage_issue(const GemvDev &a, Staged<B, NV> &r) {
-    if constexpr (NV == 0) { (void)a; (void)r; return; } else {
+    if constexpr (NV == 0) { (void)a; (void)r; return; } else
+    if constexpr (CW != 0) {
+        static_assert(ROLE == R_RESID_COMBINE && B == 1, "CW: the one-sequence combine role");
+        cw_issue<NV>(a, r);
+    } else {
     const uint32_t tid = threadIdx.x, nthr = a.nthr, n = a.n;
     const bool plain = !has_flag<ROLE>(a, F_PRE) && !has_flag<ROLE>(a, F_COMBINE);
     const __amdgpu_buffer_rsrc_t rx = mkrsrc(a.xin, plain ? ((a.nb - 1) * a.xin_bstride + n) * 4u : 0u);
diff --git a/nano_amd/csrc/gemv_q80.hip b/nano_amd/csrc/gemv_q80.hip
--- a/nano_amd/csrc/gemv_q80.hip
+++ b/nano_amd/csrc/gemv_q80.hip
@@ -134,6 +134,7 @@
             lds = n16 + ng4 * 4 + 64 + comb + slab_unit_table(d, nch);
         }
     }
+    p.cw = (a.gs == 64 && B == 1 && p.role == R_RESID_COMBINE && p.nv == 1 && p.variant != Q80_VAR_EARLY && combine_wave_shape(a)) ? 1u : 0u;
     if (lds > GEMV_Q80_LDS_MAX) return false;
     p.lds_bytes = (uint32_t)lds;
     if (out) *out = p;
diff --git a/nano_amd/csrc/gemv_q80_host.h b/nano_amd/csrc/gemv_q80_host.h
--- a/nano_amd/csrc/gemv_q80_host.h
+++ b/nano_amd/csrc/gemv_q80_host.h
@@ -25,6 +25,11 @@
     if (d.n % 1024u || d.n < 2048u || d.n > 4096u || d.ng * 64u != d.n) return 0u;
     return d.n / 1024u;
 }
+static inline bool combine_wave_shape(const GemvArgs &a) {
+    if (!a.attn_part || a.attn_table || a.nb != 1u || a.attn_nsplit == 0u || a.attn_nsplit > 8u) return false;
+    const uint32_t hd = a.attn_hd;
+    return (hd == 32u || hd == 64u || hd == 128u || hd == 256u) && (uint64_t)a.attn_n_head * hd == a.n;
+}
 static inline size_t slab_unit_table(const GemvDev &d, uint32_t nch) { return (size_t)(d.tpw * 4) * (nch <= 2u ? 4u : 8u) * 4u; }
 
 extern hipEvent_t g_q80_probe_start, g_q80_probe_stop;
diff --git a/nano_amd/csrc/gemv_q80_impl.h b/nano_amd/csrc/gemv_q80_impl.h
--- a/nano_amd/csrc/gemv_q80_impl.h
+++ b/nano_amd/csrc/gemv_q80_impl.h
@@ -12,7 +12,7 @@
     *reinterpret_cast<uint32_t *>(dst) = q80_pack4(q80_quant4(v, scale));
 }
 
-template <int ROLE, int GS, int B, int NV>
+template <int ROLE, int GS, int B, int NV, int CW = 0>
 __device__ __forceinline__ void stage_finish(const GemvDev &a, Staged<B, NV> &r, int8_t *xq, float *xs, float *red, uint32_t n16, uint32_t ng4) {
     const uint32_t tid = threadIdx.x, nthr = a.nthr, n = a.n, ng = a.ng;
     const uint32_t lane = tid & 63u, wid = tid >> 6, NW = nthr >> 6;
@@ -61,6 +61,9 @@
         }
         __syncthreads();
     } else {
+        if constexpr (CW != 0) {
+            cw_combine<NV>(a, r);
+        } else
         if (comb) {
             if constexpr (B == 1) {
                 const bool pre_ml = a.attn_n_head * 8u <= nthr;
@@ -303,69 +306,45 @@
 struct Wo13Args { GemvDev wo; GemvDev w13; SlabHand hand; uint32_t wo_wgs, wait16; };
 template <int ROLE_A, int WF, int WFA>
 __global__ __launch_bounds__(512) void wo_w13_fused_kernel(const Wo13Args fa) {
+#define WO13_CW 0
+#include "wo_w13_fused_body.inc"
+#undef WO13_CW
+}
+template <int NV, int UPW, int WFC>
+__global__ __launch_bounds__(1024) void gemv_q80_slab_cw_kernel(const GemvDev a) {
+    static_assert(NV == 1, "one item per thread (gemv_q80_plan)");
     extern __shared__ __attribute__((aligned(16))) unsigned char smem[];
-    constexpr int GS = 64, B = 1, NV = 1, UPW = 1;
-    const uint2 tk_ = hand_tick(fa.hand);
-    {
-        constexpr int ROLE = ROLE_A;
+    constexpr int ROLE = R_RESID_COMBINE, GS = 64, B = 1;
+#define SLAB_CW 1
+#define SLAB_WFC WFC
+#define SLAB_A a
 #define SLAB_BID blockIdx.x
-#define SLAB_A fa.wo
-#define SLAB_HAND 1
-#define SLAB_HANDV fa.hand
-#define SLAB_PTAG hand_ptag(tk_, fa.hand)
+#define SLAB_HAND 0
+#define SLAB_HANDV (SlabHand{})
+#define SLAB_PTAG 0u
 #define SLAB_XHAND 0
 #define SLAB_XHANDV (SlabHand{})
 #define SLAB_CTAG 0u
-#define SLAB_WFC WFA
-#define SLAB_PART 1
+#define SLAB_PART 0
 #include "gemv_q80_slab_body.inc"
-#undef SLAB_PART
-        auto wo_rest = [&]() __attribute__((always_inline)) {
-#define SLAB_PART 2
-#include "gemv_q80_slab_body.inc"
-#undef SLAB_PART
-        };
-#undef SLAB_WFC
 #undef SLAB_A
+#undef SLAB_BID
 #undef SLAB_HAND
 #undef SLAB_HANDV
 #undef SLAB_PTAG
 #undef SLAB_XHAND
 #undef SLAB_XHANDV
 #undef SLAB_CTAG
-        {
-            constexpr int ROLE = R_NORM_SWIGLU;
-#define SLAB_A fa.w13
-#define SLAB_HAND 0
-#define SLAB_HANDV (SlabHand{})
-#define SLAB_PTAG 0u
-#define SLAB_XHAND 1
-#define SLAB_XHANDV fa.hand
-#define SLAB_CTAG hand_ctag(tk_, fa.hand)
-#define SLAB_XHAND_WAIT (blockIdx.x >= fa.wo_wgs ? fa.wait16 : 0u)
-#define SLAB_XHAND_NAP 2
-#define SLAB_WF WF
-#define SLAB_PART 1
-#include "gemv_q80_slab_body.inc"
 #undef SLAB_PART
-            if (blockIdx.x < fa.wo_wgs) wo_rest();
-            __syncthreads();
-#define SLAB_PART 2
-#include "gemv_q80_slab_body.inc"
-#undef SLAB_PART
-#undef SLAB_A
-#undef SLAB_HAND
-#undef SLAB_HANDV
-#undef SLAB_PTAG
-#undef SLAB_XHAND
-#undef SLAB_XHANDV
-#undef SLAB_CTAG
-#undef SLAB_XHAND_WAIT
-#undef SLAB_XHAND_NAP
-#undef SLAB_WF
-        }
-#undef SLAB_BID
-    }
+#undef SLAB_WFC
+#undef SLAB_CW
+}
+template <int WF, int WFA>
+__global__ __launch_bounds__(512) void wo_w13_fused_cw_kernel(const Wo13Args fa) {
+    constexpr int ROLE_A = R_RESID_COMBINE;
+#define WO13_CW 1
+#include "wo_w13_fused_body.inc"
+#undef WO13_CW
 }
 
 #endif
@@ -509,6 +488,21 @@
         hipLaunchKernelGGL((gemv_q80_slab_kernel<ROLE, GS, B, NV, UPW, 0, 1>), dim3(p.grid), dim3(64 * p.nw), lds, st, dd);
         return hipGetLastError();
     }
+#if NANO_Q80_GS == 64
+    if constexpr (GS == 64 && B == 1 && ROLE == R_RESID_COMBINE && NV == 1) if (p.cw) {
+        if (p.variant == Q80_VAR_PLAIN) {
+            auto kern = &gemv_q80_slab_cw_kernel<NV, UPW, 0>;
+            if (lds > 64 * 1024) (void)hipFuncSetAttribute(reinterpret_cast<const void *>(kern), hipFuncAttributeMaxDynamicSharedMemorySize, (int)lds);
+            hipLaunchKernelGGL(kern, dim3(p.grid), dim3(64 * p.nw), lds, st, dd); return hipGetLastError();
+        }
+        if constexpr (UPW <= 2) {
+            if (p.variant == Q80_VAR_WFC2) { hipLaunchKernelGGL((gemv_q80_slab_cw_kernel<NV, UPW, 2>), dim3(p.grid), dim3(64 * p.nw), lds, st, dd); return hipGetLastError(); }
+            if (p.variant == Q80_VAR_WFC3) { hipLaunchKernelGGL((gemv_q80_slab_cw_kernel<NV, UPW, 3>), dim3(p.grid), dim3(64 * p.nw), lds, st, dd); return hipGetLastError(); }
+            if (p.variant == Q80_VAR_WFC4) { hipLaunchKernelGGL((gemv_q80_slab_cw_kernel<NV, UPW, 4>), dim3(p.grid), dim3(64 * p.nw), lds, st, dd); return hipGetLastError(); }
+        }
+        return hipErrorInvalidValue;
+    }
+#endif
     if constexpr (GS == 64 && B == 1 && (ROLE == R_RESID || ROLE == R_RESID_COMBINE) && (NV == 1 || NV == 2) && UPW <= 2) {
         if (p.variant == Q80_VAR_WFC2) { hipLaunchKernelGGL((gemv_q80_slab_kernel<ROLE, GS, B, NV, UPW, 0, 0, 2>), dim3(p.grid), dim3(64 * p.nw), lds, st, dd); return hipGetLastError(); }
         if (p.variant == Q80_VAR_WFC3) { hipLaunchKernelGGL((gemv_q80_slab_kernel<ROLE, GS, B, NV, UPW, 0, 0, 3>), dim3(p.grid), dim3(64 * p.nw), lds, st, dd); return hipGetLastError(); }
@@ -623,10 +617,10 @@
     d.wg_c0 = 0xffffffffu; d.wg_c1 = 0xffffffffu;
     d.nthr = nthr;
 }
-static size_t slab_lds(const GemvDev &d, bool table = true) {
+static size_t slab_lds(const GemvDev &d, bool table = true, bool wgt = true) {
     const uint32_t nmat = d.epi == GEMV_EPI_SWIGLU ? 2 : 1;
     const size_t n16 = (d.n + 15) & ~15u, ng4 = (d.ng + 3) & ~3u, pitch = ((d.ng + 47) / 64) * 64 + 16;
-    return n16 + ng4 * 4 + 64 + ((d.flags & F_COMBINE) ? (size_t)d.attn_n_head * 32 : 0) + (table ? (size_t)nmat * (d.tpw * 4) * pitch * 4 : 0);
+    return n16 + ng4 * 4 + 64 + ((d.flags & F_COMBINE) && wgt ? (size_t)d.attn_n_head * 32 : 0) + (table ? (size_t)nmat * (d.tpw * 4) * pitch * 4 : 0);
 }
 static bool wo13_shape(const GemvArgs &wo, const GemvArgs &w13, WoW13FusedPlan &f, GemvDev &da, GemvDev &db) {
     Wo13Plan q;
@@ -636,7 +630,8 @@
     const bool wf = slab_wave_fold(db);
     if (wf) db.units = (db.rw + 1) / 2;
     const bool wfa = slab_wave_fold_chunks(da) == 2u;
-    const size_t la = slab_lds(da, !wfa) + (wfa ? slab_unit_table(da, 2u) : 0), lb = slab_lds(db, !wf), lds = la > lb ? la : lb;
+    const bool cw = (da.flags & F_COMBINE) && combine_wave_shape(wo);
+    const size_t la = slab_lds(da, !wfa, !cw) + (wfa ? slab_unit_table(da, 2u) : 0), lb = slab_lds(db, !wf), lds = la > lb ? la : lb;
     if (lds > FUSED_LDS_MAX) return false;
     f = WoW13FusedPlan{};
     f.sig = 3; f.threads = 512;
@@ -645,6 +640,7 @@
     f.nv_a = 1; f.upw_a = 1; f.nv_b = 1; f.upw_b = 1;
     f.wa = q.wa; f.wb = q.wb; f.lds_bytes = (uint32_t)lds;
     f.rw_a = q.a.rw; f.rw_b = q.b.rw;
+    f.cw = cw ? 1u : 0u;
     return true;
 }
 
@@ -719,6 +715,11 @@
     h.base[0] = 0; h.base[1] = 0; h.base[2] = 0;
     fa.hand = h;
     const size_t lds = q.lds_bytes;
+#define WO13_CW_GO(WF_, WFC_) do { if (q.cw && q.role == (uint32_t)R_RESID_COMBINE && q.wf == WF_ && q.wfc == WFC_) { \
+        hipLaunchKernelGGL((wo_w13_fused_cw_kernel<WF_, WFC_>), dim3(q.wb), dim3(q.threads), lds, st, fa); return hipGetLastError(); } } while (0)
+    WO13_CW_GO(0, 0); WO13_CW_GO(0, 2); WO13_CW_GO(1, 0); WO13_CW_GO(1, 2);
+#undef WO13_CW_GO
+    if (q.cw) return hipErrorInvalidValue;
 #define WO13_GO(RA_, WF_, WFC_) do { if (q.role == (uint32_t)RA_ && q.wf == WF_ && q.wfc == WFC_) { \
         hipLaunchKernelGGL((wo_w13_fused_kernel<RA_, WF_, WFC_>), dim3(q.wb), dim3(q.threads), lds, st, fa); return hipGetLastError(); } } while (0)
     WO13_GO(R_RESID, 0, 0); WO13_GO(R_RESID, 0, 2); WO13_GO(R_RESID, 1, 0); WO13_GO(R_RESID, 1, 2);
diff --git a/nano_amd/csrc/gemv_q80_slab_body.inc b/nano_amd/csrc/gemv_q80_slab_body.inc
--- a/nano_amd/csrc/gemv_q80_slab_body.inc
+++ b/nano_amd/csrc/gemv_q80_slab_body.inc
@@ -9,6 +9,10 @@
 #ifndef SLAB_EARLY
 #define SLAB_EARLY 0
 #define SLAB_EARLY_DEFAULTED 1
+#endif
+#ifndef SLAB_CW
+#define SLAB_CW 0
+#define SLAB_CW_DEFAULTED 1
 #endif
 #ifndef SLAB_XHAND_WAIT
 #define SLAB_XHAND_WAIT 0u
@@ -74,7 +78,9 @@
     int8_t *xq = reinterpret_cast<int8_t *>(smem);
     float *xs = reinterpret_cast<float *>(smem + B * n16);
     float *red = xs + B * ng4;
-    float *P = red + B * 16 + (has_flag<ROLE>(SLAB_A, F_COMBINE) ? B * SLAB_A.attn_n_head * 8 : 0);
+    constexpr bool CW_ = (SLAB_CW) != 0;
+    static_assert(!CW_ || (ROLE == R_RESID_COMBINE && B == 1 && NV >= 1 && !(SLAB_XHAND)), "SLAB_CW: the one-sequence combine role, items in registers");
+    float *P = red + B * 16 + (!CW_ && has_flag<ROLE>(SLAB_A, F_COMBINE) ? B * SLAB_A.attn_n_head * 8 : 0);
 
     karg_touch(SLAB_A.out[0]); karg_touch(SLAB_A.out_bstride[0]); karg_touch(SLAB_A.out_pstride[0]); karg_touch(SLAB_A.rows[0]); karg_touch(SLAB_A.magic_rw); karg_touch(SLAB_A.nb);
     if (!(ROLE == R_RESID || ROLE == R_RESID_COMBINE || ROLE == R_NORM_SWIGLU)) {
@@ -86,7 +92,7 @@
     NANO_STAMP(SLAB_A.stamps, 0, tid);
     Staged<B, NV> sx;
     if constexpr (SLAB_XHAND) stage_issue_nw<ROLE, B, NV>(SLAB_A, sx);
-    else if (!(NANO_STAMPS && (SLAB_A.dbg & 2u))) stage_issue<ROLE, B, NV>(SLAB_A, sx);
+    else if (!(NANO_STAMPS && (SLAB_A.dbg & 2u))) stage_issue<ROLE, B, NV, (SLAB_CW)>(SLAB_A, sx);
 
     constexpr bool ONESEG = ROLE == R_RESID || ROLE == R_RESID_COMBINE || ROLE == R_NORM_SWIGLU;
     const int sel = (ONESEG || swiglu) ? 0 : (int)(SLAB_BID >= SLAB_A.wg_c0) + (int)(SLAB_BID >= SLAB_A.wg_c1);
@@ -104,7 +110,7 @@
     static_assert(SLAB_PART == 0 || early_ == 0u, "SLAB_EARLY: the whole body only");
 #pragma unroll
     for (int k = 0; k < UPW; k++) { if (early_ == 0u || (uint32_t)k < early_) SLAB_ISSUE_UNIT(k); }
-    if (!SLAB_XHAND && NANO_STAMPS && (SLAB_A.dbg & 2u)) stage_issue<ROLE, B, NV>(SLAB_A, sx);
+    if (!SLAB_XHAND && NANO_STAMPS && (SLAB_A.dbg & 2u)) stage_issue<ROLE, B, NV, (SLAB_CW)>(SLAB_A, sx);
     const int fb = (int)(((uint32_t)tid * SLAB_A.magic_rw) >> 16);
     const int frl = tid - fb * (int)RW;
     const bool fold_live = tid < (int)(RW * B) && fb < (int)SLAB_A.nb && lrow0 + frl < rows0;
@@ -147,7 +153,7 @@
         }
         if (!got_) hand_give_up(SLAB_XHANDV, SLAB_A.err);
     }
-    stage_finish<ROLE, GS, B, NV>(SLAB_A, sx, xq, xs, red, n16, ng4);
+    stage_finish<ROLE, GS, B, NV, (SLAB_CW)>(SLAB_A, sx, xq, xs, red, n16, ng4);
     if constexpr (early_ != 0u) {
 #pragma unroll
         for (int k = 1; k < UPW; k++) { if ((uint32_t)k >= early_) SLAB_ISSUE_UNIT(k); }
@@ -362,6 +368,10 @@
 #undef SLAB_EARLY
 #undef SLAB_EARLY_DEFAULTED
 #endif
+#ifdef SLAB_CW_DEFAULTED
+#undef SLAB_CW
+#undef SLAB_CW_DEFAULTED
+#endif
 #ifdef SLAB_XHAND_WAIT_DEFAULTED
 #undef SLAB_XHAND_WAIT
 #undef SLAB_XHAND_NAP
diff --git a/nano_amd/csrc/kernels.h b/nano_amd/csrc/kernels.h
--- a/nano_amd/csrc/kernels.h
+++ b/nano_amd/csrc/kernels.h
@@ -40,7 +40,8 @@
     float *f32_scratch; size_t f32_scratch_floats;
     const float *attn_part;
     const float *attn_ml;
-    uint32_t attn_nsplit, attn_n_head, attn_hd, _pad2;
+    uint32_t attn_nsplit, attn_n_head, attn_hd;
+    uint32_t attn_table;
     const float *resid_add; uint32_t resid_add_bstride, _pad3;
     float *tile_max;
     uint32_t cus;
@@ -90,6 +91,7 @@
     uint32_t rw, nw, grid, lds_bytes;
     uint32_t variant, pre;
     uint32_t early, units, wg_c0, wg_c1;
+    uint32_t cw;
 };
 bool gemv_q80_plan(const GemvArgs &a, Q80GemvPlan *p);
 uint32_t gemv_q80_fit_batch(const GemvArgs &a);
@@ -220,6 +222,7 @@
     uint32_t nv_a, upw_a, nv_b, upw_b;
     uint32_t wa, wb, lds_bytes;
     uint32_t rw_a, rw_b;
+    uint32_t cw;
 };
 bool wo_w13_fused_plan(const GemvArgs &wo, const GemvArgs &w13, WoW13FusedPlan *p);
 inline bool wo_w13_fused_supports(const GemvArgs &wo, const GemvArgs &w13) { return wo_w13_fused_plan(wo, w13, nullptr); }
diff --git a/nano_amd/csrc/ops.hip b/nano_amd/csrc/ops.hip
--- a/nano_amd/csrc/ops.hip
+++ b/nano_amd/csrc/ops.hip
@@ -366,6 +366,7 @@
     a.epi = d.kind == 0 ? GEMV_EPI_STORE : d.kind == 1 ? GEMV_EPI_RESID : GEMV_EPI_SWIGLU;
     a.norm_w = d.norm_w;
     if (d.attn_part) { a.attn_part = d.attn_part; a.attn_nsplit = d.attn_nsplit; a.attn_n_head = d.attn_n_head; a.attn_hd = d.attn_hd; }
+    if (d.attn_part) { const char *cwv = getenv("NANO_COMBINE_WAVE"); a.attn_table = (cwv && *cwv == '0') ? 1u : 0u; }
     if (d.resid_add) { a.resid_add = d.resid_add; a.resid_add_bstride = d.resid_add_stride; }
     a.ordered = d.ordered ? 1u : 0u;
     r.quant = d.quant; r.cus = (int)a.cus; r.mfma_min_nb = (d.use_gemm && d.quant == NANO_QUANT_Q80) ? 1u : 9u;
@@ -445,7 +446,8 @@
         return 0;
     }
     if (k == ROUTE_GEMV_PREQ) { a.xq_in = L.r.gq; a.xs_in = L.r.gxs; a.norm_w = nullptr; }
-    return report_first_slice<NANO_Q80_GEMV_PLAN_WORDS>(L, out, gemv_q80_plan, [k](const Q80GemvPlan &p) {
+    return report_first_slice<NANO_Q80_GEMV_PLAN_WORDS>(L, out, gemv_q80_plan, [k, out](const Q80GemvPlan &p) {
+        out[16] = p.cw;
         return Words<13>{{ k, p.kernel, p.role, p.gs, p.B, p.nv, p.upw, p.rw, p.nw, p.grid, p.lds_bytes, p.variant, p.pre }}; });
 }
 
@@ -796,7 +798,7 @@
     memcpy(out, v, sizeof(v));
 }
 static void plan_words(const WoW13FusedPlan &p, uint32_t *out) {
-    const uint32_t v[NANO_WO_W13_FUSED_PLAN_WORDS] = { p.sig, p.threads, p.role, p.wf, p.wfc, p.nv_a, p.upw_a, p.nv_b, p.upw_b, p.wa, p.wb, p.lds_bytes, p.rw_a, p.rw_b, 0u, 1u };
+    const uint32_t v[NANO_WO_W13_FUSED_PLAN_WORDS] = { p.sig, p.threads, p.role, p.wf, p.wfc, p.nv_a, p.upw_a, p.nv_b, p.upw_b, p.wa, p.wb, p.lds_bytes, p.rw_a, p.rw_b, 0u, 1u, p.cw };
     memcpy(out, v, sizeof(v));
 }
 
diff --git a/nano_amd/csrc/wo_w13_fused_body.inc b/nano_amd/csrc/wo_w13_fused_body.inc
--- /dev/null
+++ b/nano_amd/csrc/wo_w13_fused_body.inc
@@ -0,0 +1,65 @@
+    extern __shared__ __attribute__((aligned(16))) unsigned char smem[];
+    constexpr int GS = 64, B = 1, NV = 1, UPW = 1;
+    const uint2 tk_ = hand_tick(fa.hand);
+    {
+        constexpr int ROLE = ROLE_A;
+#define SLAB_BID blockIdx.x
+#define SLAB_A fa.wo
+#define SLAB_HAND 1
+#define SLAB_HANDV fa.hand
+#define SLAB_PTAG hand_ptag(tk_, fa.hand)
+#define SLAB_XHAND 0
+#define SLAB_XHANDV (SlabHand{})
+#define SLAB_CTAG 0u
+#define SLAB_WFC WFA
+#define SLAB_CW WO13_CW
+#define SLAB_PART 1
+#include "gemv_q80_slab_body.inc"
+#undef SLAB_PART
+        auto wo_rest = [&]() __attribute__((always_inline)) {
+#define SLAB_PART 2
+#include "gemv_q80_slab_body.inc"
+#undef SLAB_PART
+        };
+#undef SLAB_WFC
+#undef SLAB_CW
+#undef SLAB_A
+#undef SLAB_HAND
+#undef SLAB_HANDV
+#undef SLAB_PTAG
+#undef SLAB_XHAND
+#undef SLAB_XHANDV
+#undef SLAB_CTAG
+        {
+            constexpr int ROLE = R_NORM_SWIGLU;
+#define SLAB_A fa.w13
+#define SLAB_HAND 0
+#define SLAB_HANDV (SlabHand{})
+#define SLAB_PTAG 0u
+#define SLAB_XHAND 1
+#define SLAB_XHANDV fa.hand
+#define SLAB_CTAG hand_ctag(tk_, fa.hand)
+#define SLAB_XHAND_WAIT (blockIdx.x >= fa.wo_wgs ? fa.wait16 : 0u)
+#define SLAB_XHAND_NAP 2
+#define SLAB_WF WF
+#define SLAB_PART 1
+#include "gemv_q80_slab_body.inc"
+#undef SLAB_PART
+            if (blockIdx.x < fa.wo_wgs) wo_rest();
+            __syncthreads();
+#define SLAB_PART 2
+#include "gemv_q80_slab_body.inc"
+#undef SLAB_PART
+#undef SLAB_A
+#undef SLAB_HAND
+#undef SLAB_HANDV
+#undef SLAB_PTAG
+#undef SLAB_XHAND
+#undef SLAB_XHANDV
+#undef SLAB_CTAG
+#undef SLAB_XHAND_WAIT
+#undef SLAB_XHAND_NAP
+#undef SLAB_WF
+        }
+#undef SLAB_BID
+    }
```

Result: faster. 2090 (median of 6 runs) (+1.8%).
